# nloyfer/wgbs_tools

Hardware: AMD Instinct MI355X
Metric: CpG-sites/sec segmented (higher is better)
Workload: dtype u8 counts -> u32 prefix sums -> f32/f64 log-likelihood (bit-exact with the reference)

## Files before the change

include/wgbsseg.h:

```cpp
#ifndef WGBSSEG_H
#define WGBSSEG_H

#include <stddef.h>
#include <stdint.h>

#ifdef __cplusplus
extern "C" {
#endif

#define WGBSSEG_VERSION 270
#define WGBSSEG_MAX_CPG 65535

#define WGBSSEG_OK              0
#define WGBSSEG_E_ARG          -1
#define WGBSSEG_E_METH_GT_COV  -2
#define WGBSSEG_E_NOMEM        -3
#define WGBSSEG_E_HIP          -4
#define WGBSSEG_E_LOCI_ORDER   -5
#define WGBSSEG_E_CAPACITY     -6
#define WGBSSEG_E_STATE        -7
#define WGBSSEG_E_IO           -8

typedef struct wgbsseg_ctx wgbsseg_ctx;

typedef struct wgbsseg_params {
    float    pseudo_count;
    uint32_t max_cpg;
    uint32_t max_bp;
} wgbsseg_params;

typedef struct wgbsseg_timings {
    double scan_ms;
    double window_ms;
    double cost_ms;
    double dp_ms;
    double trace_ms;
    double total_ms;
    int64_t sites;
    int64_t pairs;
    int64_t evals;
    int64_t scan_bytes;
    int32_t max_window;
    int32_t n_stages;
    int32_t scan_launches;
    int32_t div_short;
    double  scan_main_ms;
    int64_t scan_main_bytes;
} wgbsseg_timings;

int wgbsseg_version(void);

int wgbsseg_device_count(void);

int wgbsseg_create(int device, wgbsseg_ctx** out, char* err, size_t errlen);
void wgbsseg_destroy(wgbsseg_ctx* ctx);

int wgbsseg_set_betas_host(wgbsseg_ctx* ctx, const uint8_t* const* samples, int64_t n_samples, int64_t n_sites,
                           char* err, size_t errlen);
int wgbsseg_set_lbetas_host(wgbsseg_ctx* ctx, const uint16_t* const* samples, int64_t n_samples, int64_t n_sites,
                            char* err, size_t errlen);
int wgbsseg_set_betas_device(wgbsseg_ctx* ctx, const void* base, int64_t n_samples, int64_t pitch_bytes,
                             int64_t n_sites, char* err, size_t errlen);

int wgbsseg_set_loci_host(wgbsseg_ctx* ctx, const uint32_t* loci, int64_t n_sites, char* err, size_t errlen);
int wgbsseg_set_loci_device(wgbsseg_ctx* ctx, const void* loci, int64_t n_sites, char* err, size_t errlen);

int wgbsseg_segment_chunks(wgbsseg_ctx* ctx, const int64_t* chunk_start0, const int32_t* chunk_len,
                           int64_t n_chunks, const wgbsseg_params* params,
                           int32_t* borders_out, int64_t borders_cap, int64_t* borders_off,
                           char* err, size_t errlen);

int wgbsseg_segment_regions(wgbsseg_ctx* ctx, const int64_t* region_start, const int64_t* region_end, int64_t n_regions,
                            int64_t chunk_size, const wgbsseg_params* params,
                            int32_t* borders_out, int64_t borders_cap, int64_t* borders_off, int64_t* stats,
                            char* err, size_t errlen);

typedef int (*wgbsseg_batch_fn)(void* user, const int64_t* starts, const int64_t* ends, int64_t n,
                                const int32_t** out_ptr, int64_t* out_cnt);
int wgbsseg_stitch_regions(const int64_t* region_start, const int64_t* region_end, int64_t n_regions, int64_t chunk_size,
                           wgbsseg_batch_fn fn, void* user, int32_t speculate, int32_t* borders_out, int64_t borders_cap,
                           int64_t* borders_off, int64_t* stats, char* err, size_t errlen);

int wgbsseg_first_batch_items(const int64_t* region_start, const int64_t* region_end, int64_t n_regions, int64_t chunk_size,
                              int32_t speculate, int64_t* starts, int64_t* ends, int64_t cap, int64_t* n_items, int64_t* n_chunks,
                              char* err, size_t errlen);

int wgbsseg_set_site_base(wgbsseg_ctx* ctx, int64_t site_base);

typedef struct wgbsseg_group wgbsseg_group;
int wgbsseg_plan_shares(const uint32_t* loci, int64_t n_sites, const int64_t* region_start, const int64_t* region_end,
                        int64_t n_regions, int64_t chunk_size, const wgbsseg_params* params, int32_t n_shares, int64_t halo,
                        int64_t* own_lo, int64_t* own_hi, int64_t* win_lo, int64_t* win_hi, int64_t* share_chunks,
                        int64_t* share_work, char* err, size_t errlen);
int wgbsseg_plan_shares_weighted(const uint32_t* loci, int64_t n_sites, const int64_t* region_start, const int64_t* region_end,
                                 int64_t n_regions, int64_t chunk_size, const wgbsseg_params* params, int32_t n_shares, const double* weights,
                                 int64_t halo, int64_t* own_lo, int64_t* own_hi, int64_t* win_lo, int64_t* win_hi,
                                 int64_t* share_chunks, int64_t* share_work, char* err, size_t errlen);
int wgbsseg_group_create(const int32_t* devices, int32_t n_shares, wgbsseg_group** out, char* err, size_t errlen);
void wgbsseg_group_destroy(wgbsseg_group* g);
int32_t wgbsseg_group_size(const wgbsseg_group* g);
int wgbsseg_group_plan(wgbsseg_group* g, const uint32_t* loci, int64_t n_sites, const int64_t* region_start,
                       const int64_t* region_end, int64_t n_regions, int64_t chunk_size, const wgbsseg_params* params,
                       int64_t halo, int64_t* win_lo, int64_t* win_hi, int64_t* share_chunks, int64_t* share_work,
                       char* err, size_t errlen);
int wgbsseg_group_load_host(wgbsseg_group* g, const uint8_t* const* samples, int64_t n_samples, int64_t n_sites,
                            char* err, size_t errlen);
int wgbsseg_group_load_host_async(wgbsseg_group* g, const uint8_t* const* samples, int64_t n_samples, int64_t n_sites,
                                  char* err, size_t errlen);
int wgbsseg_group_load_wait(wgbsseg_group* g, char* err, size_t errlen);
int wgbsseg_group_share_set_device(wgbsseg_group* g, int32_t share, const void* base, int64_t n_samples,
                                   int64_t pitch_bytes, char* err, size_t errlen);
int wgbsseg_group_segment_regions(wgbsseg_group* g, int32_t* borders_out, int64_t borders_cap, int64_t* borders_off,
                                  int64_t* stats, char* err, size_t errlen);

int wgbsseg_group_segment_region_range(wgbsseg_group* g, int64_t first_region, int64_t end_region, int32_t* borders_out, int64_t borders_cap,
                                       int64_t* borders_off, int64_t* stats, char* err, size_t errlen);
int wgbsseg_group_get_timings(const wgbsseg_group* g, int32_t share, wgbsseg_timings* out);

int wgbsseg_segment_chunks_host(const uint8_t* betas, int64_t n_samples, int64_t sample_pitch_bytes,
                                int64_t n_sites_total, const uint32_t* loci,
                                const int64_t* chunk_start0, const int32_t* chunk_len, int64_t n_chunks,
                                const wgbsseg_params* params, int device,
                                int32_t* borders_out, int64_t borders_cap, int64_t* borders_off,
                                char* err, size_t errlen);

int wgbsseg_prefix_sums(wgbsseg_ctx* ctx, int64_t start0, int64_t len, uint32_t* out, char* err, size_t errlen);

int wgbsseg_scan_only(wgbsseg_ctx* ctx, const int64_t* chunk_start0, const int32_t* chunk_len, int64_t n_chunks,
                      int repeat, int want_carry, double* ms_per_launch, int64_t* bytes_per_launch,
                      int64_t* carry_bytes_per_launch, char* err, size_t errlen);
// ... 106 lines not shown
```

wgbs_tools_amd/_lib.py:

```python
import ctypes as C
import os
import os.path as op

import numpy as np

HERE = op.dirname(op.abspath(__file__))
LIB_PATH = op.join(HERE, 'csrc', 'libwgbsseg.so')
if os.environ.get('WGBSSEG_LIB') and os.environ.get('WGBSSEG_ALLOW_LIB_OVERRIDE') == '1':
    LIB_PATH = os.environ['WGBSSEG_LIB']
    import sys as _sys
    print('[wgbsseg] WGBSSEG_LIB: loading %s instead of the in-tree library' % LIB_PATH, file=_sys.stderr)
SYNTH_LIB_PATH = op.join(HERE, 'csrc', 'libwgbssynth.so')

OK, E_ARG, E_METH_GT_COV, E_NOMEM, E_HIP, E_LOCI_ORDER, E_CAPACITY, E_STATE, E_IO = 0, -1, -2, -3, -4, -5, -6, -7, -8

ABI_VERSION = 270
EXPORTS = ['wgbsseg_version', 'wgbsseg_device_count', 'wgbsseg_create', 'wgbsseg_destroy',
           'wgbsseg_set_betas_host', 'wgbsseg_set_betas_device', 'wgbsseg_set_loci_host', 'wgbsseg_set_loci_device',
           'wgbsseg_segment_chunks', 'wgbsseg_segment_regions', 'wgbsseg_segment_chunks_host', 'wgbsseg_prefix_sums', 'wgbsseg_scan_only',
           'wgbsseg_get_timings', 'wgbsseg_debug_fetch', 'wgbsseg_debug_sample_terms', 'wgbsseg_debug_log2',
           'wgbsseg_debug_div', 'wgbsseg_debug_check_div', 'wgbsseg_debug_div_short', 'wgbsseg_add_loci', 'wgbsseg_add_loci_borders', 'wgbsseg_block_sums', 'wgbsseg_last_block_sums_ms',
           'wgbsseg_set_site_base', 'wgbsseg_stitch_regions', 'wgbsseg_group_create', 'wgbsseg_group_destroy', 'wgbsseg_group_size',
           'wgbsseg_group_plan', 'wgbsseg_group_load_host', 'wgbsseg_group_share_set_device', 'wgbsseg_group_segment_regions', 'wgbsseg_group_segment_region_range',
           'wgbsseg_group_get_timings', 'wgbsseg_plan_shares', 'wgbsseg_set_lbetas_host',
           'wgbsseg_convert_regions', 'wgbsseg_patbeta_create', 'wgbsseg_patbeta_feed', 'wgbsseg_patbeta_finish',
           'wgbsseg_patbeta_destroy', 'wgbsseg_patbeta_kernel_ms', 'wgbsseg_group_load_host_async', 'wgbsseg_group_load_wait',
           'wgbsseg_marker_stats', 'wgbsseg_blocks_parse', 'wgbsseg_blocks_write_table', 'wgbsseg_blocks_write_bedgraph',
           'wgbsseg_format_fixed', 'wgbsseg_bed_parse', 'wgbsseg_bed_write_annotated', 'wgbsseg_debug_canonical_float',
           'wgbsseg_first_batch_items', 'wgbsseg_plan_shares_weighted',
           'wgbsseg_homog_create', 'wgbsseg_homog_feed', 'wgbsseg_homog_finish', 'wgbsseg_homog_destroy', 'wgbsseg_homog_kernel_ms',
           'wgbsseg_debug_homog_bins',
           'wgbsseg_bimodal_create', 'wgbsseg_bimodal_feed', 'wgbsseg_bimodal_finish', 'wgbsseg_bimodal_destroy', 'wgbsseg_bimodal_kernel_ms',
           'wgbsseg_debug_bimodal_terms', 'wgbsseg_sample_stats',
           'wgbsseg_pair_ranges', 'wgbsseg_pair_hist', 'wgbsseg_pair_hist_limits',
           'wgbsseg_beta2bed', 'wgbsseg_beta2bed_pass_ms', 'wgbsseg_beta2bed_limits']


class NativeLibraryError(RuntimeError):
    pass


class SegmentorError(RuntimeError):

    def __init__(self, code, msg):
        super().__init__('[wgbsseg %d] %s' % (code, msg))
        self.code = code
        self.msg = msg


class Params(C.Structure):
    _fields_ = [('pseudo_count', C.c_float), ('max_cpg', C.c_uint32), ('max_bp', C.c_uint32)]


SAMPLE_STAT_DTYPE = np.dtype([('n_sites', np.uint64), ('meth_sum', np.uint64), ('cov_sum', np.uint64), ('covered', np.uint64),
                              ('covered_at', np.uint64), ('orphans', np.uint64), ('ratio_lo', np.uint64), ('ratio_hi', np.uint64),
                              ('max_cov', np.uint32), ('reserved', np.uint32)])

PAIR_RANGE_DTYPE = np.dtype([('n', np.uint64), ('a_min', np.float64), ('a_max', np.float64), ('b_min', np.float64), ('b_max', np.float64)])


class BedOpts(C.Structure):
    _fields_ = [('min_cov', C.c_int32), ('mean', C.c_int32), ('keep_na', C.c_int32), ('stage_bytes', C.c_int32), ('slab_sites', C.c_int64)]


class Timings(C.Structure):
    _fields_ = [('scan_ms', C.c_double), ('window_ms', C.c_double), ('cost_ms', C.c_double), ('dp_ms', C.c_double),
                ('trace_ms', C.c_double), ('total_ms', C.c_double), ('sites', C.c_int64), ('pairs', C.c_int64),
                ('evals', C.c_int64), ('scan_bytes', C.c_int64), ('max_window', C.c_int32), ('n_stages', C.c_int32),
                ('scan_launches', C.c_int32), ('div_short', C.c_int32), ('scan_main_ms', C.c_double),
                ('scan_main_bytes', C.c_int64)]

    def as_dict(self):
        return {k: getattr(self, k) for k, _ in self._fields_}


BATCH_FN = C.CFUNCTYPE(C.c_int, C.c_void_p, C.POINTER(C.c_int64), C.POINTER(C.c_int64), C.c_int64, C.POINTER(C.c_void_p),
                       C.POINTER(C.c_int64))

_lib = None
_synth = None
ERRLEN = 512
_hip_preloaded = False


def _share_hip_runtime_with_torch():
    global _hip_preloaded
    if _hip_preloaded:
        return
    _hip_preloaded = True
    import importlib.util
    import sys
    if 'torch' in sys.modules:
        return
    try:
        spec = importlib.util.find_spec('torch')
    except (ImportError, ValueError):
        spec = None
    if spec is None or not spec.origin:
        return
    cand = op.join(op.dirname(spec.origin), 'lib', 'libamdhip64.so')
    if op.isfile(cand):
        try:
            C.CDLL(cand, mode=C.RTLD_GLOBAL)
        except OSError:
            pass


def load():
    global _lib
    if _lib is not None:
        return _lib
    if not op.isfile(LIB_PATH):
        raise NativeLibraryError('%s is missing: build it with `python -m wgbs_tools_amd.build` (needs hipcc). '
                                 'There is no CPU fallback.' % LIB_PATH)
    _share_hip_runtime_with_torch()
    L = C.CDLL(LIB_PATH)
    vp, i64, i32 = C.c_void_p, C.c_int64, C.c_int
    L.wgbsseg_version.restype = i32
    got = L.wgbsseg_version()
    if got != ABI_VERSION:
        raise NativeLibraryError('%s reports ABI version %d, this binding was written against %d (include/wgbsseg.h WGBSSEG_VERSION): '
                                 'rebuild it with `python -m wgbs_tools_amd.build -f`' % (LIB_PATH, got, ABI_VERSION))
    L.wgbsseg_device_count.restype = i32
    L.wgbsseg_create.restype = i32
    L.wgbsseg_create.argtypes = [i32, C.POINTER(vp), C.c_char_p, C.c_size_t]
    L.wgbsseg_destroy.restype = None
    L.wgbsseg_destroy.argtypes = [vp]
    L.wgbsseg_set_betas_host.restype = i32
    L.wgbsseg_set_betas_host.argtypes = [vp, C.POINTER(vp), i64, i64, C.c_char_p, C.c_size_t]
    L.wgbsseg_set_lbetas_host.restype = i32
    L.wgbsseg_set_lbetas_host.argtypes = [vp, C.POINTER(vp), i64, i64, C.c_char_p, C.c_size_t]
    L.wgbsseg_set_betas_device.restype = i32
    L.wgbsseg_set_betas_device.argtypes = [vp, vp, i64, i64, i64, C.c_char_p, C.c_size_t]
    L.wgbsseg_set_loci_host.restype = i32
    L.wgbsseg_set_loci_host.argtypes = [vp, vp, i64, C.c_char_p, C.c_size_t]
    L.wgbsseg_set_loci_device.restype = i32
    L.wgbsseg_set_loci_device.argtypes = [vp, vp, i64, C.c_char_p, C.c_size_t]
    L.wgbsseg_segment_chunks.restype = i32
    L.wgbsseg_segment_chunks.argtypes = [vp, vp, vp, i64, C.POINTER(Params), vp, i64, vp, C.c_char_p, C.c_size_t]
    L.wgbsseg_segment_regions.restype = i32
    L.wgbsseg_segment_regions.argtypes = [vp, vp, vp, i64, i64, C.POINTER(Params), vp, i64, vp, vp, C.c_char_p, C.c_size_t]
    L.wgbsseg_segment_chunks_host.restype = i32
    L.wgbsseg_segment_chunks_host.argtypes = [vp, i64, i64, i64, vp, vp, vp, i64, C.POINTER(Params), i32, vp, i64, vp,
                                              C.c_char_p, C.c_size_t]
    L.wgbsseg_prefix_sums.restype = i32
    L.wgbsseg_prefix_sums.argtypes = [vp, i64, i64, vp, C.c_char_p, C.c_size_t]
    L.wgbsseg_scan_only.restype = i32
    L.wgbsseg_scan_only.argtypes = [vp, vp, vp, i64, i32, i32, C.POINTER(C.c_double), C.POINTER(i64), C.POINTER(i64), C.c_char_p, C.c_size_t]
    L.wgbsseg_get_timings.restype = i32
    L.wgbsseg_get_timings.argtypes = [vp, C.POINTER(Timings)]
    L.wgbsseg_debug_fetch.restype = i64
    L.wgbsseg_debug_fetch.argtypes = [vp, C.c_char_p, vp, i64]
    L.wgbsseg_debug_sample_terms.restype = i32
# ... 941 lines not shown
```

wgbs_tools_amd/build.py:

```python
import os
import os.path as op
import shutil
import subprocess
import sys

HERE = op.dirname(op.abspath(__file__))
CSRC = op.join(HERE, 'csrc')
ARCH = 'gfx950'
HIPFLAGS = ['--offload-arch=' + ARCH, '-O3', '-std=c++17', '-ffp-contract=off', '-fPIC', '-shared', '-pthread']

TARGETS = {
    'libwgbsseg.so': (['wgbsseg.hip'], ['owners.h', 'env.h', 'seg_kernels.h', 'block_plan.h', 'block_kernels.h', 'plain_dp.h', 'wave_prims.h', 'exact_log2.h', 'stitch.h', 'add_loci.h', 'table_io.h', 'pat_kernels.h', 'homog_kernels.h', 'bimodal_kernels.h', 'stats_kernels.h', 'pair_plan.h', 'pair_kernels.h', 'bed_fmt.h', 'bed_plan.h', 'bed_kernels.h', 'share_plan.h', '../../include/wgbsseg.h']),
    'libwgbssynth.so': (['synth.hip'], []),
}


def source_hash():
    import hashlib
    srcs, hdrs = TARGETS['libwgbsseg.so']
    h = hashlib.sha256()
    for f in sorted(op.normpath(op.join(CSRC, x)) for x in srcs + hdrs):
        with open(f, 'rb') as fh:
            h.update(fh.read())
    return h.hexdigest()[:16]


def hipcc():
    for cand in (shutil.which('hipcc'), '/opt/rocm/bin/hipcc'):
        if cand and op.isfile(cand):
            return cand
    raise RuntimeError('hipcc not found: cannot build the gfx950 libraries')


PROGRAMS = {
    'segmentor': (['segmentor_main.cpp'], ['../../include/wgbsseg.h']),
}


def _stale(out, deps):
    if not op.isfile(out):
        return True
    t = op.getmtime(out)
    return any(op.getmtime(d) > t for d in deps if op.isfile(d))


def build(force=False, verbose=False):
    built = []
    for lib, (srcs, hdrs) in TARGETS.items():
        out = op.join(CSRC, lib)
        srcp = [op.join(CSRC, s) for s in srcs]
        deps = srcp + [op.normpath(op.join(CSRC, h)) for h in hdrs]
        if not all(op.isfile(s) for s in srcp):
            continue
        if force or _stale(out, deps):
            cmd = [hipcc()] + HIPFLAGS + srcp + ['-o', out]
            if verbose:
                print(' '.join(cmd), file=sys.stderr)
            subprocess.check_call(cmd, cwd=CSRC)
            built.append(lib)
    for exe, (srcs, hdrs) in PROGRAMS.items():
        out = op.join(CSRC, exe)
        srcp = [op.join(CSRC, s) for s in srcs]
        deps = srcp + [op.normpath(op.join(CSRC, h)) for h in hdrs] + [op.join(CSRC, 'libwgbsseg.so')]
        if force or _stale(out, deps):
            cmd = [hipcc(), '-O2', '-std=c++17'] + srcp + ['-L' + CSRC, '-lwgbsseg', '-Wl,-rpath,$ORIGIN', '-o', out]
            if verbose:
                print(' '.join(cmd), file=sys.stderr)
            subprocess.check_call(cmd, cwd=CSRC)
            built.append(exe)
    return built


if __name__ == '__main__':
    print(build(force='-f' in sys.argv, verbose=True))
```

wgbs_tools_amd/csrc/seg_kernels.h:

```cpp
#pragma once
#include <hip/hip_runtime.h>
#include <stddef.h>
#include <stdint.h>
#include "exact_log2.h"
#include "wave_prims.h"

#ifndef WG_CARRY_SHIFT
#define WG_CARRY_SHIFT  7
#endif
#define WG_SCAN_STAGED  512
#define WG_CARRY_G      (1 << WG_CARRY_SHIFT)
static_assert(WG_CARRY_SHIFT >= 4 && WG_CARRY_SHIFT <= 10, "k_scan: a lane vector is 16 sites, an iteration 1024");
#define WG_BLOCK        256
#define WG_WIN_TILE     1024
#define WG_PAIR_CAP     4096
#define WG_TRACE_WIN    32768
#define WG_NARROW_WMAX  60
#define WG_MEDIUM_WMAX  252
#define WG_MEDIUM_TS    16

__device__ const wg_log_tables g_wg_tables = WG_LOG_TABLES_INIT;

__device__ __forceinline__ void wg_fast_tables_to_lds(wg_fast_tables* ft, int tid, int nthreads)
{
    const double* f = reinterpret_cast<const double*>(g_wg_tables.f_tab);
    const double* d = reinterpret_cast<const double*>(g_wg_tables.d_tab);
    double* of = reinterpret_cast<double*>(ft->f_tab);
    double* od = reinterpret_cast<double*>(ft->d_fast);
    for (int x = tid; x < 32; x += nthreads) of[x] = f[x];
    for (int x = tid; x < 128; x += nthreads) {
        double v = d[x];
        if (x == 2 * WG_FAST_CENTRE_ENTRY) v = 1.0;
        if (x == 2 * WG_FAST_CENTRE_ENTRY + 1) v = 0.0;
        od[x] = v;
    }
}

__device__ __forceinline__ void wg_lookup_tables_to_lds(wg_d2* iy, wg_d2* ky, int rows, const wg_d2* __restrict__ src, int tid, int nthreads)
{
    if (src) {
        wg_d2* dst = iy;
        for (int x = tid; x < rows * (16 + 64); x += nthreads) dst[x] = src[x];
        return;
    }
    for (int x = tid; x < rows * 16; x += nthreads) iy[x] = wg_ks_iy_entry(&g_wg_tables, rows, x);
    for (int x = tid; x < rows * 64; x += nthreads) ky[x] = wg_ks_ky_entry(&g_wg_tables, rows, x);
}

struct ChunkDesc {
    int64_t start0;
    int64_t site_off;
    int64_t carry_off;
    int64_t unit_off;
    int32_t len;
    int32_t nG;
};

struct JobView {
    const uint8_t* betas;
    int64_t pitch;
    int64_t n_total;
    const uint32_t* loci;
    const ChunkDesc* chunks;
    uint2* carry;
    uint16_t* W16;
    uint32_t* cum32;
    uint16_t* back16;
    uint16_t* umax16;
    int64_t* chunk_pairs;
    int32_t n_samples;
    int32_t n_chunks;
};

struct JobStatus {
    unsigned long long first_bad;
    unsigned long long total_pairs;
    unsigned int max_window;
    unsigned int loci_disorder;
    unsigned int overflow;
    unsigned int wide_units;
};

struct StageView {
    const int64_t* cbase;
    const uint32_t* cum0;
    const int64_t* tbaseA;
    const int64_t* tbaseB;
    int32_t stage;
    const int32_t* sb;
};

__device__ __forceinline__ uint4 wg_load16_guarded(const uint8_t* row, int64_t abs_site, int64_t n_total)
{
    if (abs_site + 8 <= n_total) return *reinterpret_cast<const uint4*>(row + 2 * abs_site);
    uint32_t w[4] = {0u, 0u, 0u, 0u};
    for (int j = 0; j < 8; j++) {
        int64_t a = abs_site + j;
        if (a < n_total) {
            uint32_t m = row[2 * a], c = row[2 * a + 1];
            w[j >> 1] |= (m | (c << 8)) << (16 * (j & 1));
        }
    }
    return make_uint4(w[0], w[1], w[2], w[3]);
}

__device__ __forceinline__ void wg_sum8(const uint4 v, uint32_t& tm, uint32_t& tt, bool& anybad)
{
    const uint32_t w[4] = {v.x, v.y, v.z, v.w};
    uint32_t sm = 0, sc = 0, ok = 0x01000100u;
#pragma unroll
    for (int d = 0; d < 4; d++) {
        const uint32_t m = w[d] & 0x00ff00ffu, c = (w[d] >> 8) & 0x00ff00ffu;
        sm += m; sc += c;
        ok &= (c | 0x01000100u) - m;
    }
    tm = (sm & 0xffffu) + (sm >> 16);
    tt = (sc & 0xffffu) + (sc >> 16);
    anybad = (ok & 0x01000100u) != 0x01000100u;
}

__device__ __noinline__ uint4 wg_blank_outside(uint4 v, int rel0, int len)
{
    uint32_t w[4] = {v.x, v.y, v.z, v.w};
#pragma unroll
    for (int j = 0; j < 8; j++) {
        const int rel = rel0 + j;
        if (rel < 0 || rel >= len) w[j >> 1] &= ~(0xffffu << (16 * (j & 1)));
    }
    return make_uint4(w[0], w[1], w[2], w[3]);
}

__device__ __noinline__ int wg_first_bad_site(uint4 v0, uint4 v1)
{
    const uint32_t w[8] = {v0.x, v0.y, v0.z, v0.w, v1.x, v1.y, v1.z, v1.w};
    int bad = 16;
    for (int j = 15; j >= 0; j--) {
        const uint32_t h = w[j >> 1] >> (16 * (j & 1));
        if ((h & 0xffu) > ((h >> 8) & 0xffu)) bad = j;
    }
    return bad;
}

__global__ __launch_bounds__(WG_BLOCK) void k_scan(JobView J, JobStatus* st)
{
    const int lane = threadIdx.x & 63;
    const int64_t rowid = (int64_t)blockIdx.x * (WG_BLOCK / 64) + (threadIdx.x >> 6);
    const int64_t nrows = (int64_t)J.n_chunks * J.n_samples;
    if (rowid >= nrows) return;
    const int c = (int)(rowid / J.n_samples);
    const int s = (int)(rowid - (int64_t)c * J.n_samples);
    const ChunkDesc cd = J.chunks[c];
    const int64_t a_abs = cd.start0 & ~15LL;
    const int head = (int)(cd.start0 - a_abs);
    const int len = cd.len;
    const int span = head + len;
    const uint4* rv = reinterpret_cast<const uint4*>(J.betas + (int64_t)s * J.pitch) + (a_abs >> 3);
    const int64_t vl = ((J.n_total - 1) >> 3) - (a_abs >> 3);
    const int vlast = vl > 0x7ffffff0 ? 0x7ffffff0 : (int)vl;
    uint2* carry = J.carry + cd.carry_off + (int64_t)s * cd.nG;
    const int A6 = (int)(a_abs & (WG_CARRY_G - 1));
    uint32_t run_m = 0, run_t = 0;
    int bad_rel = 0x7fffffff;
    if (lane == 0) carry[0] = make_uint2(0u, 0u);
    const int nit = (span + 1023) >> 10;
    __shared__ uint2 cstage[WG_BLOCK / 64][WG_SCAN_STAGED];
    uint2* cs = cstage[threadIdx.x >> 6];
    const bool staged = cd.nG <= WG_SCAN_STAGED;

    int vi = 2 * lane;
    uint4 c0 = rv[vi < vlast ? vi : vlast], c1 = rv[vi + 1 < vlast ? vi + 1 : vlast];
    for (int base = 0; base < (nit << 10); base += 1024) {
        const int vn = vi + 128;
        const uint4 m0 = rv[vn < vlast ? vn : vlast], m1 = rv[vn + 1 < vlast ? vn + 1 : vlast];
// ... 202 lines not shown
        const int64_t at = cd.site_off + k0;
        const int nv = cd.len - k0 < WG_WIN_TILE ? cd.len - k0 : WG_WIN_TILE;
        tile_info[t] = make_int4((int)(uint32_t)at, (int)(at >> 32), nv, c);
    }
}

__global__ __launch_bounds__(WG_BLOCK) void k_window_scan(JobView J, JobStatus* st, const int64_t* __restrict__ wtile_off,
                                                          const uint32_t* __restrict__ tile_tot, uint32_t* __restrict__ tile_base)
{
    __shared__ uint64_t ws[WG_BLOCK / 64];
    const int tid = threadIdx.x, lane = tid & 63, wv = tid >> 6;
    const int c = blockIdx.x;
    const int64_t t0 = wtile_off[c], t1 = wtile_off[c + 1];
    uint64_t run = 0;
    for (int64_t base = t0; base < t1; base += WG_BLOCK) {
        const int64_t t = base + tid;
        const uint64_t v = t < t1 ? (uint64_t)tile_tot[t] : 0;
        const uint64_t incl = wg_wave_incl_scan_u64(v, lane);
        if (lane == 63) ws[wv] = incl;
        __syncthreads();
        uint64_t o = 0, tot = 0;
#pragma unroll
        for (int q = 0; q < WG_BLOCK / 64; q++) { if (q < wv) o += ws[q]; tot += ws[q]; }
        __syncthreads();
        if (t < t1) tile_base[t] = (uint32_t)(run + o + incl - v);
        run += tot;
    }
    if (tid == 0) {
        J.chunk_pairs[c] = (int64_t)run;
        atomicAdd(&st->total_pairs, (unsigned long long)run);
        if (run >> 32) atomicMax(&st->overflow, 1u);
    }
}

#define WG_CUM_TILES 4
__global__ __launch_bounds__(WG_BLOCK) void k_window_cum(const uint16_t* __restrict__ W16, uint32_t* __restrict__ cum32, const int4* __restrict__ tile_info,
                                                         const uint32_t* __restrict__ tile_base, int64_t n_tiles)
{
    __shared__ uint32_t ws[WG_CUM_TILES][WG_BLOCK / 64];
    const int tid = threadIdx.x, lane = tid & 63, wv = tid >> 6;
    const int64_t t0 = (int64_t)blockIdx.x * WG_CUM_TILES;
    int4 info[WG_CUM_TILES];
    uint32_t base[WG_CUM_TILES];
#pragma unroll
    for (int q = 0; q < WG_CUM_TILES; q++) {
        const int64_t t = t0 + q < n_tiles ? t0 + q : n_tiles - 1;
        info[q] = tile_info[t];
        base[q] = tile_base[t];
        if (t0 + q >= n_tiles) info[q].z = 0;
    }
    uint2 v[WG_CUM_TILES];
#pragma unroll
    for (int q = 0; q < WG_CUM_TILES; q++) {
        const int64_t at = (int64_t)(((uint64_t)(uint32_t)info[q].y << 32) | (uint32_t)info[q].x) + 4 * tid;
        v[q] = make_uint2(0u, 0u);
        if (4 * tid < info[q].z) v[q] = *reinterpret_cast<const uint2*>(W16 + at);
    }
    uint32_t w[WG_CUM_TILES][4], tot[WG_CUM_TILES], incl[WG_CUM_TILES];
#pragma unroll
    for (int q = 0; q < WG_CUM_TILES; q++) {
        const int k = 4 * tid, n = info[q].z;
        w[q][0] = k < n ? v[q].x & 0xffffu : 0u; w[q][1] = k + 1 < n ? v[q].x >> 16 : 0u;
        w[q][2] = k + 2 < n ? v[q].y & 0xffffu : 0u; w[q][3] = k + 3 < n ? v[q].y >> 16 : 0u;
        tot[q] = w[q][0] + w[q][1] + w[q][2] + w[q][3];
        incl[q] = wg_wave_incl_scan_dpp_u32(tot[q]);
        if (lane == 63) ws[q][wv] = incl[q];
    }
    __syncthreads();
#pragma unroll
    for (int q = 0; q < WG_CUM_TILES; q++) {
        const int k = 4 * tid, n = info[q].z;
        if (k >= n) continue;
        uint32_t e = base[q] + (incl[q] - tot[q]);
#pragma unroll
        for (int x = 0; x < WG_BLOCK / 64; x++) if (x < wv) e += ws[q][x];
        const int64_t at = (int64_t)(((uint64_t)(uint32_t)info[q].y << 32) | (uint32_t)info[q].x) + k;
        uint32_t* C = cum32 + at;
        const uint4 o = make_uint4(e, e + w[q][0], e + w[q][0] + w[q][1], e + w[q][0] + w[q][1] + w[q][2]);
        if (k + 4 <= n) *reinterpret_cast<uint4*>(C) = o;
        else { C[0] = o.x; if (k + 1 < n) C[1] = o.y; if (k + 2 < n) C[2] = o.z; }
    }
}

struct PlanArgs { const int32_t* sb; int32_t TI, WA, TK, n_stages, WM; };

struct TileDesc { int32_t chunk, ka, nk, et_lo; };

__device__ __forceinline__ void wg_group_tiles(const JobView& J, const ChunkDesc& cd, const PlanArgs& P, int ka, int s1,
                                               uint32_t& nA, uint32_t& nB, uint32_t& nM)
{
    const int kb = (ka + P.TI < s1) ? ka + P.TI : s1;
    uint32_t m = 0, tb = 0, tm = 0;
    for (int k0 = ka; k0 < kb; k0 += 16) {
        const uint32_t um = J.umax16[cd.unit_off + (k0 >> 4)];
        const int nk = (kb - k0 < 16) ? kb - k0 : 16;
        m = um > m ? um : m;
        if (um <= (uint32_t)P.WM) tm += 1u;
        else tb += ((uint32_t)(nk - 1) + um + (uint32_t)P.TK - 1u) / (uint32_t)P.TK;
    }
    const bool narrow = m <= (uint32_t)P.WA;
    nA = narrow ? 1u : 0u;
    nB = narrow ? 0u : tb;
    nM = narrow ? 0u : tm;
}

__global__ __launch_bounds__(WG_BLOCK) void k_tile_count(JobView J, PlanArgs P, uint32_t* __restrict__ cntA, uint32_t* __restrict__ cntB,
                                                         uint32_t* __restrict__ cntM)
{
    __shared__ uint32_t wa[WG_BLOCK / 64], wb[WG_BLOCK / 64], wm[WG_BLOCK / 64];
    const int tid = threadIdx.x, lane = tid & 63, wv = tid >> 6;
    const int c = blockIdx.x, stg = blockIdx.y;
    const ChunkDesc cd = J.chunks[c];
    const int s0 = P.sb[stg];
    uint32_t a = 0, b = 0, m = 0;
    if (s0 < cd.len) {
        const int s1 = (P.sb[stg + 1] < cd.len) ? P.sb[stg + 1] : cd.len;
        const int nU = (s1 - s0 + P.TI - 1) / P.TI;
        for (int u = tid; u < nU; u += WG_BLOCK) {
            uint32_t na, nb, nm;
            wg_group_tiles(J, cd, P, s0 + u * P.TI, s1, na, nb, nm);
            a += na; b += nb; m += nm;
        }
    }
    for (int o = 32; o > 0; o >>= 1) { a += (uint32_t)__shfl_down((int)a, o); b += (uint32_t)__shfl_down((int)b, o); m += (uint32_t)__shfl_down((int)m, o); }
    if (lane == 0) { wa[wv] = a; wb[wv] = b; wm[wv] = m; }
    __syncthreads();
    if (tid == 0) {
        uint32_t ta = 0, tb = 0, tm = 0;
        for (int q = 0; q < WG_BLOCK / 64; q++) { ta += wa[q]; tb += wb[q]; tm += wm[q]; }
        cntA[(int64_t)stg * J.n_chunks + c] = ta;
        cntB[(int64_t)stg * J.n_chunks + c] = tb;
        cntM[(int64_t)stg * J.n_chunks + c] = tm;
    }
}

#define WG_PLAN_BLOCK 256
__global__ __launch_bounds__(WG_PLAN_BLOCK) void k_stage_plan(JobView J, PlanArgs P, const uint32_t* __restrict__ cntA,
                                                         const uint32_t* __restrict__ cntB, const uint32_t* __restrict__ cntM, int64_t* cbase, uint32_t* cum0,
                                                         int64_t* tbaseA, int64_t* tbaseB, int64_t* tbaseM, int64_t* stage_pairs, int64_t* stage_tiles)
{
    __shared__ uint64_t wa[WG_PLAN_BLOCK / 64], wb[WG_PLAN_BLOCK / 64], wc[WG_PLAN_BLOCK / 64], wd[WG_PLAN_BLOCK / 64];
    const int tid = threadIdx.x, lane = tid & 63, wv = tid >> 6;
    const int stg = blockIdx.x;
    const int nC = J.n_chunks;
    uint64_t runA = 0, runB = 0, runC = 0, runD = 0;
    for (int base = 0; base < nC; base += WG_PLAN_BLOCK) {
        const int c = base + tid;
        uint64_t sz = 0, nt = 0, nu = 0, nm = 0;
        uint32_t c0 = 0;
        if (c < nC) {
            const ChunkDesc cd = J.chunks[c];
            const int64_t s0 = P.sb[stg];
            if (s0 < cd.len) {
                const int64_t s1 = (P.sb[stg + 1] < cd.len) ? P.sb[stg + 1] : cd.len;
                c0 = J.cum32[cd.site_off + s0];
                const uint64_t cend = (s1 < cd.len) ? (uint64_t)J.cum32[cd.site_off + s1] : (uint64_t)J.chunk_pairs[c];
                sz = cend - c0;
                nt = cntA ? (uint64_t)cntA[(int64_t)stg * nC + c] : (uint64_t)((s1 - s0 + P.TI - 1) / P.TI);
                nu = cntA ? (uint64_t)cntB[(int64_t)stg * nC + c] : 0;
                nm = cntA ? (uint64_t)cntM[(int64_t)stg * nC + c] : 0;
            }
        }
        const uint64_t ia = wg_wave_incl_scan_u64(sz, lane), ib = wg_wave_incl_scan_u64(nt, lane), ic = wg_wave_incl_scan_u64(nu, lane),
                       id = wg_wave_incl_scan_u64(nm, lane);
        if (lane == 63) { wa[wv] = ia; wb[wv] = ib; wc[wv] = ic; wd[wv] = id; }
        __syncthreads();
        uint64_t oa = 0, ob = 0, oc = 0, od = 0, ta = 0, tb2 = 0, tc = 0, td = 0;
#pragma unroll
        for (int q = 0; q < WG_PLAN_BLOCK / 64; q++) {
            if (q < wv) { oa += wa[q]; ob += wb[q]; oc += wc[q]; od += wd[q]; }
            ta += wa[q]; tb2 += wb[q]; tc += wc[q]; td += wd[q];
        }
        __syncthreads();
        if (c < nC) {
            cbase[(int64_t)stg * nC + c] = (int64_t)(runA + oa + ia - sz);
            cum0[(int64_t)stg * nC + c] = c0;
            tbaseA[(int64_t)stg * (nC + 1) + c] = (int64_t)(runB + ob + ib - nt);
            tbaseB[(int64_t)stg * (nC + 1) + c] = (int64_t)(runC + oc + ic - nu);
            tbaseM[(int64_t)stg * (nC + 1) + c] = (int64_t)(runD + od + id - nm);
        }
        runA += ta; runB += tb2; runC += tc; runD += td;
    }
    if (tid == 0) {
        tbaseA[(int64_t)stg * (nC + 1) + nC] = (int64_t)runB;
        tbaseB[(int64_t)stg * (nC + 1) + nC] = (int64_t)runC;
        tbaseM[(int64_t)stg * (nC + 1) + nC] = (int64_t)runD;
        stage_pairs[stg] = (int64_t)runA;
        stage_tiles[3 * stg] = (int64_t)runB;
        stage_tiles[3 * stg + 1] = (int64_t)runC;
        stage_tiles[3 * stg + 2] = (int64_t)runD;
    }
}

__global__ __launch_bounds__(WG_BLOCK) void k_tile_emit(JobView J, PlanArgs P, int stg, const int64_t* __restrict__ tbaseA,
                                                        const int64_t* __restrict__ tbaseB, const int64_t* __restrict__ tbaseM,
                                                        TileDesc* __restrict__ tilesA, TileDesc* __restrict__ tilesB, TileDesc* __restrict__ tilesM)
{
    __shared__ uint32_t wa[WG_BLOCK / 64], wb[WG_BLOCK / 64], wm[WG_BLOCK / 64];
    const int tid = threadIdx.x, lane = tid & 63, wv = tid >> 6;
    const int c = blockIdx.x;
    const int nC = J.n_chunks;
    const ChunkDesc cd = J.chunks[c];
    const int s0 = P.sb[stg];
    if (s0 >= cd.len) return;
    const int s1 = (P.sb[stg + 1] < cd.len) ? P.sb[stg + 1] : cd.len;
    const int nU = (s1 - s0 + P.TI - 1) / P.TI;
    int64_t runA = tbaseA[(int64_t)stg * (nC + 1) + c], runB = tbaseB[(int64_t)stg * (nC + 1) + c], runM = tbaseM[(int64_t)stg * (nC + 1) + c];
    for (int base = 0; base < nU; base += WG_BLOCK) {
        const int u = base + tid;
        const int ka = s0 + u * P.TI;
        uint32_t na = 0, nb = 0, nm = 0;
        if (u < nU) wg_group_tiles(J, cd, P, ka, s1, na, nb, nm);
        const uint32_t ia = wg_wave_incl_scan_dpp_u32(na), ib = wg_wave_incl_scan_dpp_u32(nb), im = wg_wave_incl_scan_dpp_u32(nm);
        if (lane == 63) { wa[wv] = ia; wb[wv] = ib; wm[wv] = im; }
        __syncthreads();
        uint32_t oa = 0, ob = 0, om = 0, ta = 0, tb = 0, tm = 0;
#pragma unroll
        for (int q = 0; q < WG_BLOCK / 64; q++) { if (q < wv) { oa += wa[q]; ob += wb[q]; om += wm[q]; } ta += wa[q]; tb += wb[q]; tm += wm[q]; }
        __syncthreads();
        if (u < nU) {
            const int kb = (ka + P.TI < s1) ? ka + P.TI : s1;
            if (na) {
                TileDesc d = {c, ka, kb - ka, 0};
                tilesA[runA + oa + ia - na] = d;
            } else {
                int64_t o = runB + ob + ib - nb, om2 = runM + om + im - nm;
                for (int k0 = ka; k0 < kb; k0 += 16) {
                    const uint32_t um = J.umax16[cd.unit_off + (k0 >> 4)];
                    const int nk = (kb - k0 < 16) ? kb - k0 : 16;
                    if (um <= (uint32_t)P.WM) { TileDesc d = {c, k0, nk, 0}; tilesM[om2++] = d; continue; }
                    const int kt = (int)(((uint32_t)(nk - 1) + um + (uint32_t)P.TK - 1u) / (uint32_t)P.TK);
                    for (int e = 0; e < kt; e++) { TileDesc d = {c, k0, nk, k0 + e * P.TK}; tilesB[o++] = d; }
                }
            }
        }
        runA += ta; runB += tb; runM += tm;
    }
}

struct CostArgs {
    float pc, pc2;
    int32_t NS;
    int32_t rows;
    const wg_d2* tab;
    int32_t xcd_group;
    int32_t cmap;
    uint32_t* finished;
};

__global__ __launch_bounds__(64) void k_stage_gate(const uint32_t* __restrict__ finished, uint32_t need, long long max_ticks)
{
    if (threadIdx.x != 0) return;
    const long long t0 = wall_clock64();
    while (__hip_atomic_load(finished, __ATOMIC_RELAXED, __HIP_MEMORY_SCOPE_AGENT) < need && wall_clock64() - t0 < max_ticks) __builtin_amdgcn_s_sleep(8);
}

__device__ __forceinline__ void wg_stage_prefix_row(uint2* __restrict__ dst, const uint8_t* __restrict__ row,
                                                    const uint2* __restrict__ carry, const ChunkDesc& cd,
                                                    int64_t n_total, int A, int x0, int cnt0, int lane)
{
    const int cnt = x0 + cnt0;
    const int64_t abs0 = cd.start0 + A;
    const uint2 c0 = carry[(abs0 >> WG_CARRY_SHIFT) - (cd.start0 >> WG_CARRY_SHIFT)];
    uint32_t run_m = c0.x, run_t = c0.y;
    const int64_t al = abs0 & ~3LL;
    const int hs = (int)(abs0 - al);
    for (int p0 = 0; p0 < cnt + hs; p0 += 256) {
        const int sidx = p0 + lane * 4;
        const int64_t a = al + sidx;
        uint32_t w0 = 0, w1 = 0;
        if (sidx < cnt + hs) {
            if (a + 4 <= n_total) {
                const uint2 v = *reinterpret_cast<const uint2*>(row + 2 * a);
                w0 = v.x; w1 = v.y;
            } else {
                for (int j = 0; j < 4; j++) if (a + j < n_total) {
                    const uint32_t h = (uint32_t)row[2 * (a + j)] | ((uint32_t)row[2 * (a + j) + 1] << 8);
                    if (j < 2) w0 |= h << (16 * j); else w1 |= h << (16 * (j - 2));
                }
            }
        }
        uint32_t m[4], t[4];
        uint32_t tot = 0;
#pragma unroll
        for (int j = 0; j < 4; j++) {
            const uint32_t h = ((j < 2) ? w0 : w1) >> (16 * (j & 1));
            const int x = sidx + j - hs;
            const bool in = x >= 0 && (A + x) < cd.len;
// ... 626 lines not shown
    "v_cmp_gt_f64 vcc, v[6:7], v[2:3]\n"                \
    "v_max_f64 v[2:3], v[2:3], v[6:7]\n"                \
    "v_cndmask_b32_e32 v4, v4, v45, vcc\n"              \
    "v_readlane_b32 s20, v2, %[" P "]\n"                \
    "v_readlane_b32 s21, v3, %[" P "]\n"                \
    "v_add_u32_e32 v45, 1, v45\n"
#define WG_DP32W_MOVE  "v_cndmask_b32_e64 v2, v2, v42, s[24:25]\n" "v_cndmask_b32_e64 v3, v3, v43, s[24:25]\n" "v_cndmask_b32_e64 v4, v4, v44, s[24:25]\n"
#define WG_DP32W_REARM "v_cndmask_b32_e64 v42, v42, 0, s[24:25]\n" "v_cndmask_b32_e64 v43, v43, v40, s[24:25]\n"
#define WG_DP32W_CAPT  "v_cndmask_b32_e64 v5, v5, v4, s[24:25]\n"
#define WG_DP32W_BLOCK(R0, R1, R2, R3, R4, R5, R6, R7)                                                     \
            WG_DP32W_CORE(R0, "p0") WG_DP32W_MOVE                                                          \
            WG_DP32W_CORE(R1, "p1") WG_DP32W_REARM                                                         \
            WG_DP32W_CORE(R2, "p2") WG_DP64L_MASK("ml0", "mh0")                                            \
            WG_DP32W_CORE(R3, "p3") WG_DP32W_CAPT                                                          \
            WG_DP32W_CORE(R4, "p4") WG_DP32W_MOVE                                                          \
            WG_DP32W_CORE(R5, "p5") WG_DP32W_REARM                                                         \
            WG_DP32W_CORE(R6, "p6") WG_DP64L_MASK("ml1", "mh1")                                            \
            WG_DP32W_CORE(R7, "p7") WG_DP32W_CAPT
#define WG_DP32W_OPERANDS(V0, V1, V2, V3, V4, V5, V6, V7)                                                  \
            : "+{v[2:3]}"(best), "+{v4}"(arg), "+{v5}"(tbk), "+{s[20:21]}"(Mk), "+{s[24:25]}"(mask), "+{v45}"(kk), "+{v[42:43]}"(bestB), "+{v44}"(argB) \
            : V0(cur[0]), V1(cur[1]), V2(cur[2]), V3(cur[3]), V4(cur[4]), V5(cur[5]), V6(cur[6]), V7(cur[7]), "{v40}"(ninf_splat), \
              [p0] "n"(G + 0), [p1] "n"(G + 1), [p2] "n"(G + 2), [p3] "n"(G + 3), [p4] "n"(G + 4), [p5] "n"(G + 5), [p6] "n"(G + 6), [p7] "n"(G + 7), \
              [ml0] "n"((int)(uint32_t)(0xfull << G)), [mh0] "n"((int)(uint32_t)((0xfull << G) >> 32)),   \
              [ml1] "n"((int)(uint32_t)(0xfull << (G + 4))), [mh1] "n"((int)(uint32_t)((0xfull << (G + 4)) >> 32)) \
            : "v6", "v7", "vcc"

template <int G, int SET>
__device__ __forceinline__ void wg_dp_group32w(double& best, int32_t& arg, double& bestB, int32_t& argB, uint32_t& tbk, double& Mk, uint64_t& mask,
                                               uint32_t& kk, const double (&cur)[8], const uint32_t ninf_splat)
{
    if (SET == 0) asm volatile(WG_DP32W_BLOCK("v[8:9]", "v[10:11]", "v[12:13]", "v[14:15]", "v[16:17]", "v[18:19]", "v[20:21]", "v[22:23]")
                               WG_DP32W_OPERANDS("{v[8:9]}", "{v[10:11]}", "{v[12:13]}", "{v[14:15]}", "{v[16:17]}", "{v[18:19]}", "{v[20:21]}", "{v[22:23]}"));
    else          asm volatile(WG_DP32W_BLOCK("v[24:25]", "v[26:27]", "v[28:29]", "v[30:31]", "v[32:33]", "v[34:35]", "v[36:37]", "v[38:39]")
                               WG_DP32W_OPERANDS("{v[24:25]}", "{v[26:27]}", "{v[28:29]}", "{v[30:31]}", "{v[32:33]}", "{v[34:35]}", "{v[36:37]}", "{v[38:39]}"));
}

template <int STP0>
__device__ __forceinline__ void wg_dp_batch32w(double& best, int32_t& arg, double& bestB, int32_t& argB, uint32_t& tbk, double& Mk,
                                               const double* __restrict__ my, const int base, const int lane)
{
    const uint32_t ninf_hi = 0xfff00000u;
    const double NEG_INF = -__builtin_inf();
    double Ms = wg_readlane_f64(Mk, 0);
    uint32_t kk = (uint32_t)base;
    uint64_t mask = 0;
    double ra[8], rb[8];
#pragma unroll
    for (int u = 0; u < 8; u++) ra[u] = my[u * 64];
#pragma unroll
    for (int u = 0; u < 8; u++) rb[u] = my[(8 + u) * 64];
    wg_dp_group32w<STP0 + 0, 0>(best, arg, bestB, argB, tbk, Ms, mask, kk, ra, ninf_hi);
#pragma unroll
    for (int u = 0; u < 8; u++) ra[u] = my[(16 + u) * 64];
    wg_dp_group32w<STP0 + 8, 1>(best, arg, bestB, argB, tbk, Ms, mask, kk, rb, ninf_hi);
#pragma unroll
    for (int u = 0; u < 8; u++) rb[u] = my[(24 + u) * 64];
    wg_dp_group32w<STP0 + 16, 0>(best, arg, bestB, argB, tbk, Ms, mask, kk, ra, ninf_hi);
    wg_dp_group32w<STP0 + 24, 1>(best, arg, bestB, argB, tbk, Ms, mask, kk, rb, ninf_hi);
    const bool last4 = lane >= STP0 + 28 && lane < STP0 + 32;
    best = last4 ? bestB : best;
    arg = last4 ? argB : arg;
    bestB = last4 ? NEG_INF : bestB;
    Mk = Ms;
}

template <int NW, int BL, bool LEAN = false>
__global__ __launch_bounds__(64 * (1 + NW)) void k_dp(JobView J, StageView SV, const double* __restrict__ cost, DpArgs A,
                                                      double* __restrict__ state, int64_t state_stride)
{
    constexpr bool WIDEJOB = BL < 64;
    constexpr int SLOT = BL * 64 * (WIDEJOB ? 2 : 1);
    extern __shared__ __attribute__((aligned(16))) char smem_dp[];
    double* slots = reinterpret_cast<double*>(smem_dp);
    double* Mring = slots + 2 * SLOT;
    double* pendLB = Mring + 128;
    int32_t* pendLA = reinterpret_cast<int32_t*>(pendLB + 64);
    uint32_t* kinds = reinterpret_cast<uint32_t*>(pendLA + 64);
    uint32_t* metaC = kinds + 4;
    uint16_t* metaW = reinterpret_cast<uint16_t*>(metaC + WG_DP_META_RING);
    const int lane = threadIdx.x & 63;
    const int wvl = (int)(threadIdx.x >> 6);
    const bool worker = wvl != 0;
    const int lw = wvl - 1;
    const int c = blockIdx.x;
    const int nC = J.n_chunks;
    const ChunkDesc cd = J.chunks[c];
    const int s0 = SV.sb[SV.stage];
    if (s0 >= cd.len) return;
    const int s1 = (SV.sb[SV.stage + 1] < cd.len) ? SV.sb[SV.stage + 1] : cd.len;
    const int rmask = A.ringN - 1;
    double* gs = state + (int64_t)c * state_stride;
    double* pendB = gs + WG_DP_STATE_HDR;
    int32_t* pendA = reinterpret_cast<int32_t*>(pendB + A.ringN);
    const double* cb = cost + SV.cbase[(int64_t)SV.stage * nC + c];
    const uint32_t cum0 = SV.cum0[(int64_t)SV.stage * nC + c];
    const uint16_t* Wp = J.W16 + cd.site_off;
    const uint32_t* Cp = J.cum32 + cd.site_off;
    const double NEG_INF = -__builtin_inf();
    const int nb = (s1 - s0 + BL - 1) / BL;

    if (!worker) __builtin_amdgcn_s_setprio(3);
    double best = NEG_INF, bestB = NEG_INF;
    int32_t arg = 0, argB = 0;
    double Mk = 0.0;
    DpRows<NW, BL> rows;
    DpRefill<NW> refill;
    uint32_t fm_prev = 0, fm_cur = 0, fm_n1 = 0;
    constexpr int RB = WG_DP_META_REGION / BL;
    if (worker) {
        if (WIDEJOB && s0 == 0)
            for (int x = lw * 64 + lane; x < A.ringN; x += 64 * NW) pendB[x] = NEG_INF;
        wg_dp_refill_issue<NW>(refill, Wp, Cp, cum0, s0, s1, lane, lw);
        wg_dp_refill_commit<NW>(refill, metaW, metaC, 0, lane, lw);
        wg_dp_refill_issue<NW>(refill, Wp, Cp, cum0, s0 + WG_DP_META_REGION, s1, lane, lw);
        wg_dp_refill_commit<NW>(refill, metaW, metaC, WG_DP_META_REGION, lane, lw);
        if (WIDEJOB && lw == 0 && lane < BL) {
            double v = NEG_INF;
            int32_t a = 0;
            if (s0 != 0) {
                const int sl = (s0 + lane) & rmask;
                v = wg_ld_l2_f64(pendB + sl); a = wg_ld_l2_i32(pendA + sl);
                pendB[sl] = NEG_INF;
            }
            pendLB[lane] = v; pendLA[lane] = a;
        }
    } else if (s0 != 0) {
        Mk = gs[0];
        best = gs[1 + lane];
        arg = (int32_t)__double_as_longlong(gs[65 + lane]);
        if (WIDEJOB) {
            bestB = gs[129 + lane];
            argB = (int32_t)__double_as_longlong(gs[193 + lane]);
        }
        asm volatile("" : "+v"(Mk), "+v"(best), "+v"(arg), "+v"(bestB), "+v"(argB));
    }
    __syncthreads();
    if (worker) {
        wg_dp_rows_issue<NW, BL>(rows, cb, wg_dp_meta_lds<BL>(metaW, metaC, 0, lane), s0, lane, lw);
        wg_dp_rows_commit<NW, BL>(rows, slots, slots + BL * 64, kinds, lane, lw);
        fm_cur = rows.fmax;
        if (nb > 1) { wg_dp_rows_issue<NW, BL>(rows, cb, wg_dp_meta_lds<BL>(metaW, metaC, BL, lane), s0 + BL, lane, lw); fm_n1 = rows.fmax; }
    }
    __syncthreads();

#define WG_DP_BARRIER asm volatile("s_waitcnt lgkmcnt(0)\n\ts_barrier" ::: "memory")
    WG_DP_T(uint64_t dbg_wait = 0; uint64_t dbg_vm = 0; uint64_t dbg_commit = 0; uint64_t dbg_issue = 0; const uint64_t dbg_t0 = __builtin_amdgcn_s_memtime();)
    WG_DP_T(const int dbg_mode = A.pad[1];
            if (worker && (dbg_mode & 1)) return;)
    if (worker) {
      for (int b = 0; b < nb; b++) {
        const int base = s0 + b * BL;
        {
            const bool fetch = WIDEJOB && b + 1 < nb && lw == 0 && lane < BL;
            const int fsl = (base + BL + lane) & rmask;
            double fv = NEG_INF;
            int32_t fa = 0;
            if (fetch) {
                fv = wg_ld_l2_f64(pendB + fsl); fa = wg_ld_l2_i32(pendA + fsl);
                pendB[fsl] = NEG_INF;
            }
            if (b >= RB && b % RB == 0)      wg_dp_refill_issue<NW>(refill, Wp, Cp, cum0, s0 + (b / RB + 1) * WG_DP_META_REGION, s1, lane, lw);
            else if (b > RB && b % RB == 1)  wg_dp_refill_commit<NW>(refill, metaW, metaC, (b / RB + 1) * WG_DP_META_REGION, lane, lw);
            if (WIDEJOB && b >= 1 && fm_prev > 128u)
                wg_dp_far<NW, BL>(cb, Wp, Cp, cum0, base - BL, s1, Mring, pendB, pendA, rmask, lane, lw);
            WG_DP_T(const uint64_t tc0 = __builtin_amdgcn_s_memtime(); asm volatile("s_waitcnt vmcnt(0)" ::: "memory"); dbg_vm += __builtin_amdgcn_s_memtime() - tc0;)
            if (b + 1 < nb WG_DP_T(&& !(dbg_mode & 2)))
                wg_dp_rows_commit<NW, BL>(rows, slots + (size_t)((b + 1) & 1) * SLOT, slots + (size_t)((b + 1) & 1) * SLOT + BL * 64,
                                          kinds + ((b + 1) & 1), lane, lw);
            WG_DP_T(asm volatile("s_waitcnt lgkmcnt(0)" ::: "memory"); dbg_commit += __builtin_amdgcn_s_memtime() - tc0;)
            if (fetch) {
                pendLB[((b + 1) & 1) * 32 + lane] = fv;
                pendLA[((b + 1) & 1) * 32 + lane] = fa;
// ... 70 lines not shown
                else           wg_dp_wide_batch32<32>(best, arg, bestB, argB, tbk, Mfin, Mk, my, myB, base, lane);
                tbk = (uint32_t)(base + d + 1) - tbk;
                if (fin) Mring[(base + d + 1) & 127] = Mfin;
            }
            if (fin && base + d < s1) J.back16[cd.site_off + base + d] = (uint16_t)tbk;
        }
        WG_DP_T(const uint64_t tb0 = __builtin_amdgcn_s_memtime();)
        WG_DP_BARRIER;
        WG_DP_T(dbg_wait += __builtin_amdgcn_s_memtime() - tb0;)
      }
    }
#undef WG_DP_BARRIER
    WG_DP_T(if (s1 >= cd.len && lane == 0 && wvl <= 1) {
        gs[2 * wvl] = (double)(__builtin_amdgcn_s_memtime() - dbg_t0);
        gs[2 * wvl + 1] = (double)dbg_wait;
        if (wvl == 1) { gs[4] = (double)dbg_vm; gs[5] = (double)dbg_commit; gs[6] = (double)dbg_issue; }
    })
    WG_DP_T(if (s1 >= cd.len && lane == 0) {
        gs[8 + wvl] = (double)__builtin_amdgcn_s_getreg((31 << 11) | 4);
        if (wvl == 0) { gs[16] = (double)__builtin_amdgcn_s_getreg((31 << 11) | 20); gs[17] = (double)dbg_t0; gs[18] = (double)__builtin_amdgcn_s_memtime(); }
        gs[20 + wvl] = (double)dbg_wait;
        gs[40 + wvl] = (double)dbg_issue;
    })
    if (WIDEJOB && worker && fm_prev > 128u)
        wg_dp_far<NW, BL>(cb, Wp, Cp, cum0, s0 + (nb - 1) * BL, s1, Mring, pendB, pendA, rmask, lane, lw);
    if (!worker && s1 < cd.len) {
        if (lane == 0) gs[0] = Mk;
        gs[1 + lane] = best;
        gs[65 + lane] = __longlong_as_double((long long)arg);
        if (WIDEJOB) {
            gs[129 + lane] = bestB;
            gs[193 + lane] = __longlong_as_double((long long)argB);
        }
    }
}

template <int NW>
struct Dp16Rows { static constexpr int PER = (16 + NW - 1) / NW; double va[PER]; };

template <int NW>
__device__ __forceinline__ void wg_dp16_issue(Dp16Rows<NW>& R, const double* __restrict__ cb, const uint16_t* __restrict__ metaW,
                                              const uint32_t* __restrict__ metaC, int base_rel, int base, int lane, int lw)
{
    const int x = (base_rel + lane) & (WG_DP_META_RING - 1);
    const uint32_t w = lane < 16 ? (uint32_t)metaW[x] : 0u;
    const uint32_t rel = metaC[x];
    const int stp0 = base & 63;
#pragma unroll
    for (int q = 0; q < Dp16Rows<NW>::PER; q++) {
        const int sidx = lw + q * NW;
        R.va[q] = -__builtin_inf();
        if (sidx < 16) {
            const uint32_t f = (uint32_t)__builtin_amdgcn_readlane((int)w, sidx);
            const uint32_t r = (uint32_t)__builtin_amdgcn_readlane((int)rel, sidx);
            const uint32_t j = (uint32_t)(lane - stp0 - sidx) & 63u;
            if (j < f) R.va[q] = cb[(int64_t)r + j];
        }
    }
}

template <int NW>
__device__ __forceinline__ void wg_dp16_commit(const Dp16Rows<NW>& R, double* __restrict__ slot, int lane, int lw)
{
#pragma unroll
    for (int q = 0; q < Dp16Rows<NW>::PER; q++) {
        const int sidx = lw + q * NW;
        if (sidx < 16) slot[sidx * 64 + lane] = R.va[q];
    }
}

template <int NW>
__global__ __launch_bounds__(64 * (1 + NW)) void k_dp16(JobView J, StageView SV, const double* __restrict__ cost,
                                                         double* __restrict__ state, int64_t state_stride)
{
    constexpr int BL = 16, D = 4;
    constexpr int RB = WG_DP_META_REGION / BL;
    extern __shared__ __attribute__((aligned(16))) char smem_dp[];
    double* slots = reinterpret_cast<double*>(smem_dp);
    uint32_t* metaC = reinterpret_cast<uint32_t*>(slots + 2 * BL * 64);
    uint16_t* metaW = reinterpret_cast<uint16_t*>(metaC + WG_DP_META_RING);
    const int lane = threadIdx.x & 63;
    const bool worker = threadIdx.x >= 64;
    const int lw = (int)(threadIdx.x >> 6) - 1;
    const int c = blockIdx.x;
    const int nC = J.n_chunks;
    const ChunkDesc cd = J.chunks[c];
    const int s0 = SV.sb[SV.stage];
    if (s0 >= cd.len) return;
    const int s1 = (SV.sb[SV.stage + 1] < cd.len) ? SV.sb[SV.stage + 1] : cd.len;
    double* gs = state + (int64_t)c * state_stride;
    const double* cb = cost + SV.cbase[(int64_t)SV.stage * nC + c];
    const uint32_t cum0 = SV.cum0[(int64_t)SV.stage * nC + c];
    const uint16_t* Wp = J.W16 + cd.site_off;
    const uint32_t* Cp = J.cum32 + cd.site_off;
    const int nb = (s1 - s0 + BL - 1) / BL;

    if (!worker) __builtin_amdgcn_s_setprio(3);
    double best = -__builtin_inf();
    int32_t arg = 0;
    double Mk = 0.0;
    Dp16Rows<NW> r0, r1, r2, r3;
    DpRefill<NW> refill;
    if (worker) {
        wg_dp_refill_issue<NW>(refill, Wp, Cp, cum0, s0, s1, lane, lw);
        wg_dp_refill_commit<NW>(refill, metaW, metaC, 0, lane, lw);
        wg_dp_refill_issue<NW>(refill, Wp, Cp, cum0, s0 + WG_DP_META_REGION, s1, lane, lw);
        wg_dp_refill_commit<NW>(refill, metaW, metaC, WG_DP_META_REGION, lane, lw);
    } else if (s0 != 0) {
        Mk = gs[0];
        best = gs[1 + lane];
        arg = (int32_t)__double_as_longlong(gs[65 + lane]);
        asm volatile("" : "+v"(Mk), "+v"(best), "+v"(arg));
    }
    __syncthreads();
    if (worker) {
        wg_dp16_issue<NW>(r0, cb, metaW, metaC, 0, s0, lane, lw);
        wg_dp16_commit<NW>(r0, slots, lane, lw);
        if (1 < nb) wg_dp16_issue<NW>(r1, cb, metaW, metaC, 1 * BL, s0 + 1 * BL, lane, lw);
        if (2 < nb) wg_dp16_issue<NW>(r2, cb, metaW, metaC, 2 * BL, s0 + 2 * BL, lane, lw);
        if (3 < nb) wg_dp16_issue<NW>(r3, cb, metaW, metaC, 3 * BL, s0 + 3 * BL, lane, lw);
        if (4 < nb) wg_dp16_issue<NW>(r0, cb, metaW, metaC, 4 * BL, s0 + 4 * BL, lane, lw);
    }
    __syncthreads();

    const uint32_t ninf_hi = 0xfff00000u;
    uint32_t tbk = 0;
#define WG_DP16_WORKER(Q, RNEXT)                                                                                           \
    if (b4 + (Q) < nb) {                                                                                                   \
        const int b = b4 + (Q);                                                                                            \
        if (b >= RB && b % RB == 0)      wg_dp_refill_issue<NW>(refill, Wp, Cp, cum0, s0 + (b / RB + 1) * WG_DP_META_REGION, s1, lane, lw); \
        else if (b > RB && b % RB == 1)  wg_dp_refill_commit<NW>(refill, metaW, metaC, (b / RB + 1) * WG_DP_META_REGION, lane, lw); \
        if (b + 1 < nb) wg_dp16_commit<NW>(RNEXT, slots + (size_t)((b + 1) & 1) * (BL * 64), lane, lw);                       \
        if (b + 1 + D < nb) wg_dp16_issue<NW>(RNEXT, cb, metaW, metaC, (b + 1 + D) * BL, s0 + (b + 1 + D) * BL, lane, lw);     \
        asm volatile("s_waitcnt lgkmcnt(0)\n\ts_barrier" ::: "memory");                                                    \
    }
#define WG_DP16_REC(Q)                                                                                                     \
    if (b4 + (Q) < nb) {                                                                                                   \
        const int b = b4 + (Q);                                                                                            \
        const double* my = slots + (size_t)(b & 1) * (BL * 64) + lane;                                                     \
        double ra[8], rb[8];                                                                                               \
        _Pragma("unroll") for (int u = 0; u < 8; u++) { ra[u] = my[u * 64]; rb[u] = my[(8 + u) * 64]; }                    \
        double Ms = wg_readlane_f64(Mk, 0);          \
        wg_dp_group64<16 * (Q), 0>(best, arg, tbk, Ms, ra, ninf_hi);                                                       \
        wg_dp_group64<16 * (Q) + 8, 1>(best, arg, tbk, Ms, rb, ninf_hi);                                                   \
        Mk = Ms;                                                                                                           \
        asm volatile("s_waitcnt lgkmcnt(0)\n\ts_barrier" ::: "memory");                                                    \
    }
    if (worker) {
        for (int b4 = 0; b4 < nb; b4 += 4) { WG_DP16_WORKER(0, r1) WG_DP16_WORKER(1, r2) WG_DP16_WORKER(2, r3) WG_DP16_WORKER(3, r0) }
    } else {
        for (int b4 = 0; b4 < nb; b4 += 4) {
            WG_DP16_REC(0) WG_DP16_REC(1) WG_DP16_REC(2) WG_DP16_REC(3)
            const int i = s0 + b4 * BL + lane;
            const uint32_t len = (((uint32_t)lane - tbk) & 63u) + 1u;
            if (i < s1) J.back16[cd.site_off + i] = (uint16_t)len;
            tbk = 0;
        }
    }
#undef WG_DP16_WORKER
#undef WG_DP16_REC
    if (!worker && s1 < cd.len) {
        if (lane == 0) gs[0] = Mk;
        gs[1 + lane] = best;
        gs[65 + lane] = __longlong_as_double((long long)arg);
    }
}

__device__ __forceinline__ int wg_trace_step(const uint16_t* win, int i, int wlo)
{
    int stepb = (int)win[i - 1 - wlo];
    if (stepb < 1 || stepb > i) stepb = i;
    return i - stepb;
// ... 267 lines not shown
```

wgbs_tools_amd/csrc/wgbsseg.hip:

```cpp
#include <hip/hip_runtime.h>
#include <algorithm>
#include <atomic>
#include <cerrno>
#include <chrono>
#include <cstdarg>
#include <cstdio>
#include <cstdlib>
#include <cstring>
#include <deque>
#include <functional>
#include <initializer_list>
#include <memory>
#include <string>
#include <thread>
#include <vector>
#include <pthread.h>
#include <sched.h>
#include <sys/mman.h>
#include <unistd.h>
#if defined(__x86_64__) && !defined(__HIP_DEVICE_COMPILE__)
#include <emmintrin.h>
#endif

#include "../../include/wgbsseg.h"
// ... 3 lines not shown
#include "share_plan.h"
#include "block_kernels.h"
#include "pat_kernels.h"
#include "homog_kernels.h"
#include "bimodal_kernels.h"
#include "stats_kernels.h"
#include "pair_kernels.h"
#include "bed_kernels.h"
#include "plain_dp.h"
#include "stitch.h"
#include "add_loci.h"
#include "table_io.h"

namespace {

void set_err(char* err, size_t errlen, const char* fmt, ...)
{
    if (!err || !errlen) return;
    va_list ap;
    va_start(ap, fmt);
    vsnprintf(err, errlen, fmt, ap);
    va_end(ap);
}

#define HIP_TRY(expr)                                                                              \
    do {                                                                                           \
        hipError_t e__ = (expr);                                                                   \
        if (e__ != hipSuccess) {                                                                   \
            set_err(err, errlen, "HIP error %d (%s) at %s:%d: %s", (int)e__, hipGetErrorString(e__), \
                    __FILE__, __LINE__, #expr);                                                    \
            return WGBSSEG_E_HIP;                                                                  \
        }                                                                                          \
    } while (0)

hipError_t set_kernel_attributes();
inline int ceil_pow2(int v) { int r = 1; while (r < v) r <<= 1; return r; }
inline int64_t round_up(int64_t v, int64_t m) { return (v + m - 1) / m * m; }

}

#define WG_MAX_CPUS 8192
struct NearCpus { std::vector<unsigned long> bits; bool valid = false; };

enum BatchEvent { EV_BEGIN, EV_WINDOWS, EV_SCAN_END, EV_PLAN, EV_TRACE0, EV_TRACE1, EV_HOME, EV_STATS, EV_VALIDATE0, EV_VALIDATE1, EV_SCAN0, EV_SCAN1, EV_UPLOADED, EV_COUNT };

struct wgbsseg_ctx {
    int device = 0;
    NearCpus near_cpus;
    Stream sA, sB, sC;
    Stream sA2;
    DevBuf betas_own, loci_own;
    const uint8_t* betas = nullptr;
    int64_t pitch = 0, n_total = 0;
    int32_t elem = 1;
    int64_t site_base = 0;
    int32_t n_samples = 0;
    const uint32_t* loci = nullptr;
    int64_t n_loci = 0;
    DevBuf chunks, wtile, carry, W16, cum32, back16, chunk_pairs, status, tile_tot, tile_base, tile_chunk;
    DevBuf plan_cbase, plan_cum0, plan_tbase, plan_pairs, plan_tiles, plan_cnt, umax16;
    std::vector<PinnedBuf> pinned;
    std::vector<PinnedBuf> up_stage;
    DevBuf tiles[3], cost[3], stage_ctr, dpstate, tmp_borders, nb, boff, out_borders[2], edges, lookup;
    DevBuf dbg_a, dbg_b, dbg_c;
    int out_par = 0;
    Event evS;
    Event evD;
    bool out_pending = false;
    bool batch_open = false;
    std::vector<wg_d2> h_lookup;
    float lookup_pc = -1.0f;
    int lookup_rows[3] = {-1, -1, -1};
    Event ev[EV_COUNT];
    PinnedBuf h_status;
    PinnedBuf h_job, h_pieces, h_sb;
    PinnedBuf h_out;
    std::vector<Event> ev_cost0, ev_cost1, ev_dp0, ev_dp1, ev_fork, ev_join;
    wgbsseg_timings tim = {};
    int64_t last_sites = 0, last_pairs = 0;
    int32_t last_stages = 0;
    bool last_valid = false;
    long long cost_budget_bytes = 0;
    int force_stages = 0;
    bool counted_live = false;
    double stage_gate_wide_evals = 100000.0, stage_min_evals_per_step = 21000.0;
    bool stage_gate_shared = false;
    int stage_gate = 768, last_stage_pct = -1, force_dp_mode = 0, force_ns = 0, force_ti = 0;
    double last_block_sums_ms = 0.0;
    int64_t table_blocks = 0;
    bool accumulate = false;
    std::vector<std::pair<int64_t, int64_t>> validated;
    DevBuf scan_pieces, divcheck, plan_sb;
    DevBuf bs_plan, bs_desc, bs_out;
    DevBuf mk_out, cv_in, cv_out;
    DevBuf st_ranges, st_parts;
    DevBuf ph_pairs, ph_edges, ph_out;
    DevBuf bed_tab, bed_mult, bed_wg, bed_out[2];
    PinnedBuf bed_home[2], bed_tot;
    Event bed_ev[2][4];
    double bed_len_ms = 0.0, bed_emit_ms = 0.0;
    std::vector<int32_t> h_stage_bounds;
    float divs_pc = -1.0f;
    bool divs_ok = false;
    int64_t last_dp_chunks = 0, last_dp_stride = 0;
    float divs_m_pc = -1.0f;
    bool divs_m_ok = false;
    bool divs_enabled = true, bs_general = false;
    int64_t scan_piece_sites = 4096;
    int medium_wmax = WG_MEDIUM_WMAX;
    bool dp_wlean = true, early = true, speculate = true, batch_marks = false;
    ~wgbsseg_ctx() { (void)hipSetDevice(device); (void)hipDeviceSynchronize(); }
};

namespace {

bool device_local_cpus(int device, NearCpus* out)
{
    out->valid = false;
    if (!env_flag("WGBSSEG_UPLOAD_PIN", true)) return false;
    char bus[64] = {0};
    if (hipDeviceGetPCIBusId(bus, (int)sizeof bus, device) != hipSuccess) { (void)hipGetLastError(); return false; }
    for (char* q = bus; *q; q++) if (*q >= 'A' && *q <= 'F') *q = (char)(*q - 'A' + 'a');
    char path[160];
    snprintf(path, sizeof path, "/sys/bus/pci/devices/%s/local_cpulist", bus);
    FILE* f = fopen(path, "r");
    if (!f) return false;
    char line[8192] = {0};
    const bool got = fgets(line, (int)sizeof line, f) != nullptr;
    fclose(f);
    if (!got) return false;
    const size_t bytes = CPU_ALLOC_SIZE(WG_MAX_CPUS);
    std::vector<unsigned long> allowed(bytes / sizeof(unsigned long), 0ul);
    out->bits.assign(bytes / sizeof(unsigned long), 0ul);
    cpu_set_t* A = reinterpret_cast<cpu_set_t*>(allowed.data());
    cpu_set_t* L = reinterpret_cast<cpu_set_t*>(out->bits.data());
    if (sched_getaffinity(0, bytes, A) != 0) return false;
    int n_local = 0;
    for (const char* q = line; *q;) {
        while (*q == ',' || *q == ' ' || *q == '\n') q++;
        if (*q < '0' || *q > '9') break;
        char* end = nullptr;
        long a = strtol(q, &end, 10), b = a;
        if (*end == '-') b = strtol(end + 1, &end, 10);
        for (long x = a; x <= b && x < WG_MAX_CPUS; x++) if (CPU_ISSET_S((int)x, bytes, A)) { CPU_SET_S((int)x, bytes, L); n_local++; }
        q = end;
    }
    if (n_local == 0 || n_local == CPU_COUNT_S(bytes, A)) return false;
    out->valid = true;
    return true;
}
inline void pin_to(const NearCpus& n)
{
    if (n.valid) (void)pthread_setaffinity_np(pthread_self(), n.bits.size() * sizeof(unsigned long), reinterpret_cast<const cpu_set_t*>(n.bits.data()));
}
struct FillMode { bool populate = true, nt = true; };
inline void fill_piece(void* dst, const uint8_t* src, size_t n, const FillMode& m)
{
#ifdef MADV_POPULATE_READ
    if (m.populate) {
        const uintptr_t a = reinterpret_cast<uintptr_t>(src) & ~(uintptr_t)4095, b = (reinterpret_cast<uintptr_t>(src) + n + 4095) & ~(uintptr_t)4095;
        (void)madvise(reinterpret_cast<void*>(a), b - a, MADV_POPULATE_READ);
    }
#endif
#if defined(__x86_64__) && !defined(__HIP_DEVICE_COMPILE__)
    if (m.nt && (reinterpret_cast<uintptr_t>(dst) & 15) == 0) {
        __m128i* d = reinterpret_cast<__m128i*>(dst);
        const __m128i* s = reinterpret_cast<const __m128i*>(src);
        size_t v = n >> 6;
        for (; v > 0; v--, s += 4, d += 4) {
            const __m128i x0 = _mm_loadu_si128(s), x1 = _mm_loadu_si128(s + 1), x2 = _mm_loadu_si128(s + 2), x3 = _mm_loadu_si128(s + 3);
            _mm_stream_si128(d, x0); _mm_stream_si128(d + 1, x1); _mm_stream_si128(d + 2, x2); _mm_stream_si128(d + 3, x3);
        }
        _mm_sfence();
        const size_t done = n & ~(size_t)63;
        if (n > done) memcpy(static_cast<char*>(dst) + done, src + done, n - done);
        return;
    }
#endif
    memcpy(dst, src, n);
}
struct UploadPlan {
    int64_t piece = 0, ppr = 0, n_tasks = 0;
    int T = 1, depth = 2;
    bool piece_major = false;
// ... 96 lines not shown
    std::atomic<int64_t> pieces_done(0);
    std::mutex mu;
    auto complete = [&](int64_t task) {
        const int64_t p = task / n_rows;
        if (rows_done[(size_t)p].fetch_add(1) + 1 == (int)n_rows) {
            std::lock_guard<std::mutex> lk(mu);
            int64_t d = pieces_done.load();
            while (d < u.ppr && rows_done[(size_t)d].load() == (int)n_rows) d++;
            pieces_done.store(d);
            ready_sites.store(std::min<int64_t>(d * u.piece, row_bytes) / 2);
        }
    };
    const std::vector<hipError_t> terr = run_upload(c, u, dst, dst_pitch, rows, n_rows, row_bytes, complete);
    for (int t = 0; t < u.T; t++)
        if (terr[(size_t)t] != hipSuccess) { msg = std::string("HIP error during the upload: ") + hipGetErrorString(terr[(size_t)t]); return WGBSSEG_E_HIP; }
    ready_sites.store(row_bytes / 2);
    if (profiling()) fprintf(stderr, "[wgbsseg] betas to the device (streaming): %.1f ms, %.1f GB/s (%d upload threads x %d pieces of %lld KB%s%s%s)\n", (wall_s() - t0) * 1e3,
                             (double)row_bytes * n_rows / (wall_s() - t0) * 1e-9, u.T, u.depth, (long long)(u.piece >> 10), c->near_cpus.valid ? ", on the device's CPUs" : "",
                             u.fill.populate ? ", pages mapped per piece" : "", u.fill.nt ? ", non-temporal fill" : "");
    return WGBSSEG_OK;
}

}

extern "C" {

int wgbsseg_version(void) { return WGBSSEG_VERSION; }

int wgbsseg_device_count(void)
{
    int n = 0;
    if (hipGetDeviceCount(&n) != hipSuccess) return 0;
    return n;
}

}
namespace {
std::atomic<int> g_live_ctx[64];

int check_device(int device, char* err, size_t errlen)
{
    int n = 0;
    hipError_t e = hipGetDeviceCount(&n);
    if (e != hipSuccess || n <= 0) {
        set_err(err, errlen, "no HIP device available (%s); libwgbsseg has no CPU fallback", hipGetErrorString(e));
        return WGBSSEG_E_HIP;
    }
    if (device < 0 || device >= n) { set_err(err, errlen, "device %d out of range (0..%d)", device, n - 1); return WGBSSEG_E_ARG; }
    HIP_TRY(hipSetDevice(device));
    hipDeviceProp_t prop;
    HIP_TRY(hipGetDeviceProperties(&prop, device));
    if (!strstr(prop.gcnArchName, "gfx950")) {
        set_err(err, errlen, "device %d is %s; this library carries gfx950 code only", device, prop.gcnArchName);
        return WGBSSEG_E_HIP;
    }
    return WGBSSEG_OK;
}

int create_ctx(int device, bool scan_low_priority, wgbsseg_ctx** out, char* err, size_t errlen)
{
    if (!out) { set_err(err, errlen, "out is NULL"); return WGBSSEG_E_ARG; }
    *out = nullptr;
    const int rc = check_device(device, err, errlen);
    if (rc != WGBSSEG_OK) return rc;
    HIP_TRY(set_kernel_attributes());
    std::unique_ptr<wgbsseg_ctx> c(new (std::nothrow) wgbsseg_ctx());
    if (!c) { set_err(err, errlen, "out of host memory"); return WGBSSEG_E_NOMEM; }
    c->device = device;
    (void)device_local_cpus(device, &c->near_cpus);
    HIP_TRY(c->sA.create());
    {
        int lo_p = 0, hi_p = 0;
        (void)hipDeviceGetStreamPriorityRange(&lo_p, &hi_p);
        HIP_TRY(c->sB.create(hi_p));
        HIP_TRY(scan_low_priority ? c->sC.create(lo_p) : c->sC.create());
    }
    HIP_TRY(c->sA2.create());
    HIP_TRY(c->evD.create(false));
    HIP_TRY(c->evS.create(false));
    for (auto& v : c->ev) HIP_TRY(v.create());
    const long long budget_mb = env_int("WGBSSEG_COST_BUDGET_MB", 0);
    c->cost_budget_bytes = (budget_mb > 0 ? budget_mb : 6144LL) << 20;
    c->force_stages = (int)env_int("WGBSSEG_FORCE_STAGES", 0);
    c->stage_gate = (int)env_int("WGBSSEG_STAGE_GATE", c->stage_gate, 0);
    c->stage_gate_shared = env_flag("WGBSSEG_STAGE_GATE_SHARED", false);
    c->stage_gate_wide_evals = env_double("WGBSSEG_STAGE_GATE_WIDE_EVALS", c->stage_gate_wide_evals);
    c->stage_min_evals_per_step = env_double("WGBSSEG_STAGE_MIN_EVALS", c->stage_min_evals_per_step);
    if (env_int("WGBSSEG_LAST_STAGE_PCT", -1) != -1) c->last_stage_pct = (int)env_int("WGBSSEG_LAST_STAGE_PCT", -1, 5, 800);
    c->force_dp_mode = (int)env_int("WGBSSEG_DP_MODE", 0, 0, 2);
    c->force_ns = (int)env_int("WGBSSEG_NS", 0);
    c->force_ti = (int)env_int("WGBSSEG_TI", 0);
    c->bs_general = env_flag("WGBSSEG_BLOCK_SUMS_GENERAL", false);
    c->divs_enabled = env_flag("WGBSSEG_DIV_SHORT", true);
    { const long long sp = env_int("WGBSSEG_SCAN_PIECE_SITES", 0); if (sp >= 1024) c->scan_piece_sites = sp & ~1023LL; }
    const int wm = (int)env_int("WGBSSEG_MEDIUM_WMAX", WG_MEDIUM_WMAX, 0, WG_MEDIUM_WMAX);
    c->medium_wmax = wm > WG_NARROW_WMAX ? wm : 0;
    c->dp_wlean = env_flag("WGBSSEG_DP_WLEAN", true);
    c->early = !env_flag("WGBSSEG_NO_EARLY", false);
    c->speculate = !env_flag("WGBSSEG_NO_SPECULATION", false);
    c->batch_marks = env_int("WGBSSEG_PROFILE", 0) >= 2;
    g_live_ctx[device & 63].fetch_add(1, std::memory_order_relaxed);
    c->counted_live = true;
    *out = c.release();
    return WGBSSEG_OK;
}
}
extern "C" {

int wgbsseg_create(int device, wgbsseg_ctx** out, char* err, size_t errlen) { return create_ctx(device, true, out, err, errlen); }

void wgbsseg_destroy(wgbsseg_ctx* c)
{
    if (!c) return;
    if (c->counted_live) g_live_ctx[c->device & 63].fetch_sub(1, std::memory_order_relaxed);
    const double t0 = wall_s();
    delete c;
    if (profiling()) fprintf(stderr, "[wgbsseg] destroy: %.1f ms\n", (wall_s() - t0) * 1e3);
}

static hipError_t own_rows(wgbsseg_ctx* c, int64_t n_samples, int64_t n_sites, int elem)
{
    const int64_t pitch = round_up(2 * elem * n_sites, 256) + 256;
    const hipError_t e = c->betas_own.ensure((size_t)pitch * (size_t)n_samples);
    if (e != hipSuccess) return e;
    c->betas = c->betas_own.as<uint8_t>();
    c->pitch = pitch; c->n_total = n_sites; c->n_samples = (int32_t)n_samples; c->elem = elem;
    c->last_valid = false;
    return hipSuccess;
}

static int set_rows_host(wgbsseg_ctx* c, const uint8_t* const* samples, int64_t n_samples, int64_t n_sites, int elem, char* err, size_t errlen)
{
    if (!c || !samples || n_samples < 1 || n_sites < 1) { set_err(err, errlen, "bad arguments to set_betas_host"); return WGBSSEG_E_ARG; }
    for (int64_t s = 0; s < n_samples; s++)
        if (!samples[s]) { set_err(err, errlen, "samples[%lld] is NULL", (long long)s); return WGBSSEG_E_ARG; }
    HIP_TRY(hipSetDevice(c->device));
    HIP_TRY(own_rows(c, n_samples, n_sites, elem));
    return upload_rows(c, c->betas_own.as<uint8_t>(), c->pitch, samples, n_samples, 2 * elem * n_sites, "betas", err, errlen);
}

int wgbsseg_set_betas_host(wgbsseg_ctx* c, const uint8_t* const* samples, int64_t n_samples, int64_t n_sites,
                           char* err, size_t errlen)
{
    return set_rows_host(c, samples, n_samples, n_sites, 1, err, errlen);
}

int wgbsseg_set_lbetas_host(wgbsseg_ctx* c, const uint16_t* const* samples, int64_t n_samples, int64_t n_sites,
                            char* err, size_t errlen)
{
    return set_rows_host(c, reinterpret_cast<const uint8_t* const*>(samples), n_samples, n_sites, 2, err, errlen);
}

int wgbsseg_set_betas_device(wgbsseg_ctx* c, const void* base, int64_t n_samples, int64_t pitch_bytes, int64_t n_sites,
                             char* err, size_t errlen)
{
    if (!c || !base || n_samples < 1 || n_sites < 1 || pitch_bytes < 2 * n_sites) { set_err(err, errlen, "bad arguments to set_betas_device"); return WGBSSEG_E_ARG; }
    if (((uintptr_t)base & 15) || (pitch_bytes & 15)) { set_err(err, errlen, "device betas base and pitch must be multiples of 16 bytes"); return WGBSSEG_E_ARG; }
    c->betas = reinterpret_cast<const uint8_t*>(base);
    c->pitch = pitch_bytes; c->n_total = n_sites; c->n_samples = (int32_t)n_samples; c->elem = 1;
    c->last_valid = false;
    return WGBSSEG_OK;
}

int wgbsseg_set_loci_host(wgbsseg_ctx* c, const uint32_t* loci, int64_t n_sites, char* err, size_t errlen)
{
    if (!c || !loci || n_sites < 1) { set_err(err, errlen, "bad arguments to set_loci_host"); return WGBSSEG_E_ARG; }
// ... 240 lines not shown
}

void grow_events(std::vector<Event>& v, size_t n)
{
    while (v.size() < n) { v.emplace_back(); (void)v.back().create(); }
}

typedef std::function<int32_t*(int64_t)> BorderAlloc;

struct EarlyOut {
    int64_t n_lead = 0;
    bool dest_device_visible = false;
    const int32_t* edges = nullptr;
    bool pending = false;
};
int wait_pending_output(wgbsseg_ctx* c, char* err, size_t errlen)
{
    if (!c->out_pending) return WGBSSEG_OK;
    c->out_pending = false;
    HIP_TRY(hipSetDevice(c->device));
    HIP_TRY(hipEventSynchronize(c->evD));
    return WGBSSEG_OK;
}

int plain_segment_chunk(wgbsseg_ctx* c, int64_t start0, int32_t n, const wgbsseg_params* P, std::vector<int32_t>& borders, char* err, size_t errlen)
{
    const int32_t W = (int32_t)std::min<int64_t>(P->max_cpg, n);
    int64_t budget_rows = std::max<int64_t>((int64_t)W + 255, (1LL << 30) / ((int64_t)W * 8));
    const long long cap_rows = env_int("WGBSSEG_PLAIN_RING_ROWS", 0);
    if (cap_rows > 0) budget_rows = std::max<int64_t>((int64_t)W, (int64_t)cap_rows);
    const int32_t R = (int32_t)std::min<int64_t>(n, budget_rows);
    const int32_t band = R >= n ? n : R - (W - 1);
    DevBuf buf, M, T, bad;
    if (buf.ensure((size_t)W * (size_t)R * 8) != hipSuccess || M.ensure((size_t)(n + 1) * 8) != hipSuccess || T.ensure((size_t)(n + 1) * 4) != hipSuccess ||
        bad.ensure(8) != hipSuccess) {
        (void)hipGetLastError();
        set_err(err, errlen, "out of device memory for the plain recurrence of a chunk with non-ascending loci (%d sites, max_cpg %d)", (int)n, (int)W);
        return WGBSSEG_E_NOMEM;
    }
    JobStatus st = {};
    st.first_bad = ~0ULL;
    HIP_TRY(hipMemcpyAsync(bad.p, &st.first_bad, 8, hipMemcpyHostToDevice, c->sA));
    PlainArgs A = {c->betas, c->pitch, c->n_total, c->n_samples, c->loci, start0, n, W, P->max_bp, P->pseudo_count, P->pseudo_count + P->pseudo_count,
                   R, buf.as<double>(), M.as<double>(), T.as<int32_t>(), bad.as<unsigned long long>()};
    for (int32_t b0 = 0; b0 < n; b0 += band) {
        const int32_t b1 = (int32_t)std::min<int64_t>(n, (int64_t)b0 + band);
        hipLaunchKernelGGL(k_plain_rows, dim3((unsigned)((b1 - b0 + WG_BLOCK - 1) / WG_BLOCK)), dim3(WG_BLOCK), 0, c->sA, A, b0, b1);
        HIP_TRY(hipGetLastError());
        hipLaunchKernelGGL(k_plain_dp, dim3(1), dim3(WG_BLOCK), 0, c->sA, A, b0, b1);
        HIP_TRY(hipGetLastError());
    }
    std::vector<int32_t> hT((size_t)n + 1);
    HIP_TRY(hipMemcpyAsync(hT.data(), T.p, (size_t)(n + 1) * 4, hipMemcpyDeviceToHost, c->sA));
    HIP_TRY(hipMemcpyAsync(&st.first_bad, bad.p, 8, hipMemcpyDeviceToHost, c->sA));
    HIP_TRY(hipStreamSynchronize(c->sA));
    if (st.first_bad != ~0ULL) return report_bad_site(c, st, err, errlen);
    borders.clear();
    int32_t i = n;
    borders.push_back(i);
    while (i > 0) {
        const int32_t t = hT[(size_t)i];
        const int32_t nx = t > 0 ? t : 0;
        if (nx >= i) { set_err(err, errlen, "internal: back-pointer %d at step %d of a plain recurrence", (int)t, (int)i); return WGBSSEG_E_STATE; }
        i = nx;
        borders.push_back(i);
    }
    std::reverse(borders.begin(), borders.end());
    return WGBSSEG_OK;
}


struct BatchPlan {
    int Wmax = 0;
    int WA = 0;
    int WMED = 0;
    int term_mode[3] = {};
    int rows[3] = {};
    int TI = 64;
    int NS[3] = {1, 1, 1};
    size_t lds[3] = {};
    int n_stages = 1;
    bool gated = false;
    int last_pct = 100;
    const int32_t* sb = nullptr;
    bool all_narrow = false;
    std::vector<int64_t> stage_pairs, stage_tiles;
    int dp_mode = 0;
    int ringN = 0; int64_t state_stride = 0;
    int nbuf = 1;
};

size_t cost_lds(const BatchPlan& p, int ti, int cls, int ns)
{
    const int wm = cls == 2 ? WG_MEDIUM_WMAX : WG_NARROW_WMAX;
    const size_t rows = cls == 1 ? ((((size_t)ns * (WG_WIDE_TK + 1 + WG_WIDE_TS + 1) + 1) & ~(size_t)1) * 8)
                                 : ((((size_t)ns * (ti + wm + 1) + 3) & ~(size_t)3) * 4);
    const size_t tabs = p.term_mode[cls] == 2 ? (size_t)p.rows[cls] * (16 + 64) * sizeof(wg_d2) : sizeof(wg_fast_tables);
    return tabs + rows + (size_t)(ti + 1) * 16 + 32 + (cls == 1 ? 0 : ((size_t)ti * wm >> 3) + 8);
}

int plan_tiles(const wgbsseg_ctx* c, const Job& job, const JobStatus& st, float pc, BatchPlan& p, char* err, size_t errlen)
{
    p.Wmax = (int)st.max_window;
    p.WA = std::min(p.Wmax, WG_NARROW_WMAX);
    p.WMED = c->medium_wmax;
    const int tmA = wg_term_mode(pc);
    const int tmB = (tmA == 2 && 255.0 * std::max(p.Wmax, 1) >= 0x1p21) ? 1 : tmA;
    p.term_mode[0] = p.term_mode[2] = tmA;
    p.term_mode[1] = tmB;
    p.rows[0] = tmA == 2 ? wg_lookup_rows(pc, 255.0 * WG_NARROW_WMAX) : 0;
    p.rows[1] = tmB == 2 ? wg_lookup_rows(pc, 255.0 * std::max(p.Wmax, 1)) : 0;
    p.rows[2] = tmA == 2 ? wg_lookup_rows(pc, 255.0 * WG_MEDIUM_WMAX) : 0;
    if (p.rows[0] > WG_KY_KMIN + 1 || p.rows[1] > WG_KY_KMIN + 1 || p.rows[2] > WG_KY_KMIN + 1) {
        set_err(err, errlen, "internal: %d / %d / %d lookup rows", p.rows[0], p.rows[1], p.rows[2]);
        return WGBSSEG_E_ARG;
    }
    const int Nsmp = (int)c->n_samples;
    const double Favg = (double)(int64_t)st.total_pairs / (double)std::max<int64_t>(1, job.sites);
    const int ti128_max_n = 16;
    double best = -1;
    for (int ti = 128; ti >= 16; ti >>= 1) {
        if (c->force_ti > 0 && ti != c->force_ti) continue;
        for (int ns : {Nsmp, 32, 16, 8, 4}) {
            if (ns > Nsmp) continue;
            if (ti == 128 && (ns != Nsmp || (c->force_ti != 128 && Nsmp > ti128_max_n))) continue;
            if (c->force_ns > 0 && ns != std::min(c->force_ns, Nsmp)) continue;
            const size_t l = cost_lds(p, ti, 0, ns);
            if (l > 64 * 1024) continue;
            const int wgs = (int)std::min<size_t>(ti == 128 ? 8 : 5, (160 * 1024) / (size_t)round_up((int64_t)l, 1280));
            const double q = ti * std::min<double>(Favg, p.WA), eff = q / (256.0 * std::ceil(q / 256.0));
            const double groups = std::ceil((double)Nsmp / ns);
            const double score = wgs * eff / (1.0 + 0.02 * (groups - 1)) * (1.0 + 0.04 * (ti / 16));
            if (score > best) { best = score; p.TI = ti; p.NS[0] = ns; }
        }
    }
    if (best < 0) { p.TI = 16; p.NS[0] = 1; }
    auto pick_ns = [&](int cls, int ti, int max_wgs, bool forced) {
        int pick = 1;
        double top = -1;
        for (int ns : {Nsmp, 32, 16, 8, 4, 1}) {
            if (ns > Nsmp) continue;
            if (forced && c->force_ns > 0 && ns != std::min(c->force_ns, Nsmp)) continue;
            const size_t l = cost_lds(p, ti, cls, ns);
            if (l > 64 * 1024) continue;
            const int wgs = (int)std::min<size_t>(max_wgs, (160 * 1024) / (size_t)round_up((int64_t)l, 1280));
            const double score = wgs / (1.0 + 0.02 * (std::ceil((double)Nsmp / ns) - 1));
            if (score > top) { top = score; pick = ns; }
        }
        return pick;
    };
    p.NS[1] = pick_ns(1, WG_WIDE_TS, 4, true);
    p.NS[2] = pick_ns(2, WG_MEDIUM_TS, 5, false);
    const int tile_ti[3] = {p.TI, WG_WIDE_TS, WG_MEDIUM_TS};
    for (int k = 0; k < 3; k++) p.lds[k] = (size_t)round_up((int64_t)cost_lds(p, tile_ti[k], k, p.NS[k]), 16);
    return WGBSSEG_OK;
}

void plan_stages(wgbsseg_ctx* c, const Job& job, const JobStatus& st, BatchPlan& p)
{
    const int64_t total_pairs = (int64_t)st.total_pairs;
    const long long bytes = total_pairs * 8;
    int n_stages = (int)std::max<long long>(1, (bytes + c->cost_budget_bytes - 1) / c->cost_budget_bytes);
    int n_long = 0;
    for (const ChunkDesc& d : job.h) n_long += d.len >= 8192;
    const bool worth = (double)total_pairs * c->n_samples >= (double)job.max_len * c->stage_min_evals_per_step;
    if (job.max_len >= 8192) n_stages = std::max(n_stages, n_long <= 160 && worth ? 8 : 1);
    if (c->force_stages > 0) n_stages = c->force_stages;
    n_stages = std::min<int>(n_stages, std::max(1, (job.max_len + 63) / 64));
    p.all_narrow = p.Wmax <= WG_NARROW_WMAX;
    const double evals_per_step = (double)total_pairs * c->n_samples / std::max<double>(1.0, (double)job.max_len);
    p.gated = c->stage_gate > 0 && n_stages > 1 && (p.all_narrow || evals_per_step >= c->stage_gate_wide_evals || c->stage_gate_shared) &&
              (c->stage_gate_shared || g_live_ctx[c->device & 63].load(std::memory_order_relaxed) == 1);
    p.last_pct = !p.gated ? 100 : (c->last_stage_pct > 0 ? c->last_stage_pct : (evals_per_step <= 52500.0 ? 300 : 100));
    const double parts = n_stages > 1 ? (double)(n_stages - 1) + p.last_pct / 100.0 : 1.0;
    const int S = (int)round_up((int64_t)std::ceil((double)job.max_len / parts), 64);
    n_stages = std::min<int>(n_stages, (job.max_len + S - 1) / S);
    std::vector<int32_t>& sb = c->h_stage_bounds;
    sb.resize((size_t)n_stages + 1);
    for (int q = 0; q < n_stages; q++) sb[(size_t)q] = (int32_t)std::min<int64_t>((int64_t)q * S, job.max_len);
    sb[(size_t)n_stages] = (int32_t)job.max_len;
    p.sb = sb.data();
    p.n_stages = n_stages;
    p.stage_pairs.assign((size_t)n_stages, 0);
    p.stage_tiles.assign((size_t)n_stages * 3, 0);
    if (p.all_narrow) {
        for (int stg = 0; stg < n_stages; stg++) {
            int64_t nt = 0, sites_in = 0;
            for (const ChunkDesc& d : job.h) {
                const int64_t s0 = sb[(size_t)stg], s1 = std::min<int64_t>(sb[(size_t)stg + 1], d.len);
                if (s1 > s0) { nt += (s1 - s0 + p.TI - 1) / p.TI; sites_in += s1 - s0; }
            }
            p.stage_tiles[3 * (size_t)stg] = nt;
            p.stage_pairs[(size_t)stg] = n_stages == 1 ? total_pairs : std::min<int64_t>(total_pairs, sites_in * std::max(p.Wmax, 1));
        }
    }
    p.nbuf = n_stages > 1 ? (p.gated && n_stages > 2 ? 3 : 2) : 1;
    p.dp_mode = std::max(p.Wmax > 512 ? 2 : (p.Wmax > 64 ? 1 : 0), c->force_dp_mode);
    p.ringN = p.dp_mode ? ceil_pow2(p.Wmax + 128) : 0;
    p.state_stride = round_up(WG_DP_STATE_HDR + (int64_t)p.ringN + (p.ringN + 1) / 2, 2);
}

int queue_div_check(wgbsseg_ctx* c, float pc, int wmax, void* dst, char* err, size_t errlen)
{
    HIP_TRY(c->divcheck.ensure(4));
    HIP_TRY(hipMemsetAsync(c->divcheck.p, 0, 4, c->sA));
    const int max_total = 255 * wmax;
    hipLaunchKernelGGL(k_check_div, dim3((unsigned)max_total + 1), dim3(WG_BLOCK), 0, c->sA, pc, pc + pc, max_total, c->divcheck.as<unsigned int>());
    HIP_TRY(hipGetLastError());
    HIP_TRY(hipMemcpyAsync(dst, c->divcheck.p, 4, hipMemcpyDeviceToHost, c->sA));
    return WGBSSEG_OK;
}

struct Batch {
    wgbsseg_ctx* c = nullptr;
    const int64_t* chunk_start0 = nullptr; const int32_t* chunk_len = nullptr; int64_t n_chunks = 0;
    const BorderAlloc* alloc = nullptr; int64_t* borders_off = nullptr; EarlyOut* early = nullptr;
    bool allow_plain = true;
    wgbsseg_params P = {};
    Job job;
    int nC = 0; int64_t J = 0;
    JobStatus* hst = nullptr;
    JobStatus st = {};
    BatchPlan plan;
    CostArgs ca[3];
    std::vector<int64_t> tile0[3];
    DevBuf* outb = nullptr; size_t out_head = 0;
    bool marks = false;
    double hm[8] = {0, 0, 0, 0, 0, 0, 0, 0};
    void mark(int i) { if (marks) hm[i] = wall_s(); }

    int front(char* err, size_t errlen);
    int disorder_exit(char* err, size_t errlen);
    int tile_plan(char* err, size_t errlen);
    int stages(char* err, size_t errlen);
    int deliver(char* err, size_t errlen);
    int timings(char* err, size_t errlen);
};

int segment_chunks_impl(wgbsseg_ctx* c, const int64_t* chunk_start0, const int32_t* chunk_len, int64_t n_chunks,
                        const wgbsseg_params* P, const BorderAlloc& alloc, int64_t* borders_off, char* err, size_t errlen, bool allow_plain = true, EarlyOut* early = nullptr)
{
    if (!P || !borders_off) { set_err(err, errlen, "NULL params/borders pointer"); return WGBSSEG_E_ARG; }
    if (P->max_bp == 0) { set_err(err, errlen, "max_bp must be >= 1 (the reference reads uninitialised loci when it is 0: segmentor.cpp:38,114)"); return WGBSSEG_E_ARG; }
    if (P->max_cpg < 1) { set_err(err, errlen, "max_cpg must be >= 1"); return WGBSSEG_E_ARG; }
    int32_t longest = 1;
    if (chunk_len) for (int64_t i = 0; i < n_chunks; i++) longest = std::max(longest, chunk_len[i]);
    Batch b;
    b.c = c; b.chunk_start0 = chunk_start0; b.chunk_len = chunk_len; b.n_chunks = n_chunks;
    b.alloc = &alloc; b.borders_off = borders_off; b.early = early; b.allow_plain = allow_plain;
    b.P = *P;
    b.P.max_cpg = std::min<uint32_t>(P->max_cpg, (uint32_t)longest);
    if ((uint64_t)b.P.max_cpg * 255u >= (1u << 24) || b.P.max_cpg > WGBSSEG_MAX_CPG) {
        set_err(err, errlen, "max_cpg %u with chunks of up to %d sites unsupported: blocks of more than %d sites (255 * sites >= 2^24) do not keep their counts exact "
                "in the float sums of the reference itself (segmentor.cpp:122-123), and windows are stored in 16 bits", P->max_cpg, (int)longest, WGBSSEG_MAX_CPG);
        return WGBSSEG_E_ARG;
    }
    b.marks = c && c->batch_marks;
    b.mark(0);
    if (!(P->pseudo_count >= 0.0f)) { set_err(err, errlen, "pseudo_count must be >= 0"); return WGBSSEG_E_ARG; }
    if (c && c->batch_open) {
        HIP_TRY(hipSetDevice(c->device));
        HIP_TRY(hipDeviceSynchronize());
        c->out_pending = false;
    }
    if (c) c->batch_open = true;
    int rc = build_job(c, chunk_start0, chunk_len, n_chunks, b.job, true, err, errlen);
    if (rc != WGBSSEG_OK) return rc;
    rc = plan_validation(c, b.job, !c->accumulate, err, errlen);
    if (rc != WGBSSEG_OK) return rc;
    c->last_valid = false;
    b.nC = (int)n_chunks;
    b.J = b.job.sites;

    rc = b.front(err, errlen);
    if (rc != WGBSSEG_OK) return rc;
    if (b.st.loci_disorder || b.st.overflow) return b.disorder_exit(err, errlen);
    rc = plan_tiles(c, b.job, b.st, b.P.pseudo_count, b.plan, err, errlen);
    if (rc != WGBSSEG_OK) return rc;
    plan_stages(c, b.job, b.st, b.plan);
// ... 80 lines not shown
    HIP_TRY(hipStreamSynchronize(c->sA));
    HIP_TRY(hipMemcpyAsync(&st2, c->status.p, sizeof(st2), hipMemcpyDeviceToHost, c->sA));
    HIP_TRY(hipStreamSynchronize(c->sA));
    if (st2.first_bad != ~0ULL) return report_bad_site(c, st2, err, errlen);
    if (!st.loci_disorder) { set_err(err, errlen, "a chunk scores more than 2^32 blocks; use a smaller chunk_size"); return WGBSSEG_E_ARG; }
    if (!allow_plain) {
        set_err(err, errlen, "internal: loci not ascending inside chunk %u (0-based sites [%lld, +%d)) of a batch that was filtered for such chunks",
                st.loci_disorder - 1, (long long)(job.h[st.loci_disorder - 1].start0 + c->site_base), (int)job.h[st.loci_disorder - 1].len);
        return WGBSSEG_E_LOCI_ORDER;
    }
    DevBuf flags;
    HIP_TRY(flags.ensure((size_t)n_chunks * 4));
    HIP_TRY(hipMemsetAsync(flags.p, 0, (size_t)n_chunks * 4, c->sA));
    hipLaunchKernelGGL(k_find_disorder, dim3((unsigned)n_chunks), dim3(WG_BLOCK), 0, c->sA, job.v, flags.as<uint32_t>());
    HIP_TRY(hipGetLastError());
    std::vector<uint32_t> hf((size_t)n_chunks);
    HIP_TRY(hipMemcpyAsync(hf.data(), flags.p, (size_t)n_chunks * 4, hipMemcpyDeviceToHost, c->sA));
    HIP_TRY(hipStreamSynchronize(c->sA));
    std::vector<int64_t> os, ooff;
    std::vector<int32_t> ol, ob;
    for (int64_t i = 0; i < n_chunks; i++) if (!hf[(size_t)i]) { os.push_back(chunk_start0[i]); ol.push_back(chunk_len[i]); }
    if (!os.empty()) {
        ooff.resize(os.size() + 1);
        const int rc = segment_chunks_impl(c, os.data(), ol.data(), (int64_t)os.size(), &P,
                                           [&](int64_t total) { ob.resize((size_t)std::max<int64_t>(1, total)); return ob.data(); }, ooff.data(), err, errlen, false);
        if (rc != WGBSSEG_OK) return rc;
    }
    std::vector<std::vector<int32_t>> plain((size_t)n_chunks);
    for (int64_t i = 0; i < n_chunks; i++)
        if (hf[(size_t)i]) {
            wgbsseg_params Pc = P;
            const int rc = plain_segment_chunk(c, chunk_start0[i], chunk_len[i], &Pc, plain[(size_t)i], err, errlen);
            if (rc != WGBSSEG_OK) return rc;
        }
    int64_t total = 0;
    size_t oi = 0;
    for (int64_t i = 0; i < n_chunks; i++) {
        borders_off[i] = total;
        if (hf[(size_t)i]) total += (int64_t)plain[(size_t)i].size();
        else { total += ooff[oi + 1] - ooff[oi]; oi++; }
    }
    borders_off[n_chunks] = total;
    int32_t* out = (*alloc)(total);
    if (!out) { set_err(err, errlen, "borders_out too small: need %lld ints", (long long)total); return WGBSSEG_E_CAPACITY; }
    oi = 0;
    for (int64_t i = 0; i < n_chunks; i++) {
        if (hf[(size_t)i]) memcpy(out + borders_off[i], plain[(size_t)i].data(), plain[(size_t)i].size() * 4);
        else { memcpy(out + borders_off[i], ob.data() + ooff[oi], (size_t)(ooff[oi + 1] - ooff[oi]) * 4); oi++; }
    }
    c->last_valid = false;
    return WGBSSEG_OK;
}

int Batch::tile_plan(char* err, size_t errlen)
{
    BatchPlan& p = plan;
    const float pc = P.pseudo_count;
    const int n_stages = p.n_stages;
    CostArgs base;
    memset(&base, 0, sizeof(base));
    base.pc = pc; base.pc2 = pc + pc;
    base.xcd_group = 64;
    base.cmap = 3;
    for (int k = 0; k < 3; k++) { ca[k] = base; ca[k].NS = p.NS[k]; ca[k].rows = p.rows[k]; }
    if (p.term_mode[0] == 2) {
        const bool same = c->lookup_pc == pc && c->lookup_rows[0] == p.rows[0] && c->lookup_rows[1] == p.rows[1] && c->lookup_rows[2] == p.rows[2] && c->lookup.p;
        if (!same) {
            static const wg_log_tables host_tabs = WG_LOG_TABLES_INIT;
            c->h_lookup.resize((size_t)(p.rows[0] + p.rows[1] + p.rows[2]) * 80);
            wg_d2* dst = c->h_lookup.data();
            for (int rows : p.rows) {
                for (int x = 0; x < rows * 16; x++) dst[x] = wg_ks_iy_entry(&host_tabs, rows, x);
                for (int x = 0; x < rows * 64; x++) dst[rows * 16 + x] = wg_ks_ky_entry(&host_tabs, rows, x);
                dst += (size_t)rows * 80;
            }
            HIP_TRY(c->lookup.ensure(c->h_lookup.size() * sizeof(wg_d2)));
            HIP_TRY(hipMemcpyAsync(c->lookup.p, c->h_lookup.data(), c->h_lookup.size() * sizeof(wg_d2), hipMemcpyHostToDevice, c->sA));
            c->lookup_pc = pc;
            for (int k = 0; k < 3; k++) c->lookup_rows[k] = p.rows[k];
        }
        const wg_d2* tab = c->lookup.as<wg_d2>();
        for (int k = 0; k < 3; k++) { ca[k].tab = tab; tab += (size_t)p.rows[k] * 80; }
    }
    const size_t sb_bytes = (size_t)(n_stages + 1) * 4;
    HIP_TRY(c->plan_sb.ensure(sb_bytes));
    const void* src = p.sb;
    if (c->h_sb.ensure(sb_bytes)) { memcpy(c->h_sb.p, src, sb_bytes); src = c->h_sb.p; }
    HIP_TRY(hipMemcpyAsync(c->plan_sb.p, src, sb_bytes, hipMemcpyHostToDevice, c->sA));
    HIP_TRY(c->plan_cbase.ensure((size_t)n_stages * nC * 8));
    HIP_TRY(c->plan_cum0.ensure((size_t)n_stages * nC * 4));
    HIP_TRY(c->plan_tbase.ensure((size_t)n_stages * (nC + 1) * 8 * 3));
    HIP_TRY(c->plan_cnt.ensure((size_t)n_stages * nC * 4 * 3));
    HIP_TRY(c->plan_pairs.ensure((size_t)n_stages * 8));
    HIP_TRY(c->plan_tiles.ensure((size_t)n_stages * 8 * 3));
    PlanArgs pa = {c->plan_sb.as<int32_t>(), p.TI, p.WA, WG_WIDE_TK, n_stages, p.WMED};
    uint32_t* cntA = c->plan_cnt.as<uint32_t>();
    uint32_t* cntB = cntA + (size_t)n_stages * nC;
    uint32_t* cntM = cntB + (size_t)n_stages * nC;
    int64_t* tbaseA = c->plan_tbase.as<int64_t>();
    int64_t* tbaseB = tbaseA + (size_t)n_stages * (nC + 1);
    int64_t* tbaseM = tbaseB + (size_t)n_stages * (nC + 1);
    if (!p.all_narrow) {
        hipLaunchKernelGGL(k_tile_count, dim3((unsigned)nC, (unsigned)n_stages), dim3(WG_BLOCK), 0, c->sA, job.v, pa, cntA, cntB, cntM);
        HIP_TRY(hipGetLastError());
    }
    hipLaunchKernelGGL(k_stage_plan, dim3((unsigned)n_stages), dim3(WG_PLAN_BLOCK), 0, c->sA, job.v, pa, (const uint32_t*)(p.all_narrow ? nullptr : cntA),
                       (const uint32_t*)(p.all_narrow ? nullptr : cntB), (const uint32_t*)(p.all_narrow ? nullptr : cntM),
                       c->plan_cbase.as<int64_t>(), c->plan_cum0.as<uint32_t>(), tbaseA, tbaseB, tbaseM, c->plan_pairs.as<int64_t>(), c->plan_tiles.as<int64_t>());
    HIP_TRY(hipGetLastError());
    if (!p.all_narrow) {
        const bool check_div_m = c->divs_enabled && p.term_mode[2] == 2 && p.WMED > 0 && c->divs_m_pc != pc;
        int rc;
        if (check_div_m && (rc = queue_div_check(c, pc, WG_MEDIUM_WMAX, hst + 3, err, errlen)) != WGBSSEG_OK) return rc;
        HIP_TRY(hipMemcpyAsync(p.stage_pairs.data(), c->plan_pairs.p, (size_t)n_stages * 8, hipMemcpyDeviceToHost, c->sA));
        HIP_TRY(hipMemcpyAsync(p.stage_tiles.data(), c->plan_tiles.p, (size_t)n_stages * 24, hipMemcpyDeviceToHost, c->sA));
        HIP_TRY(hipStreamSynchronize(c->sA));
        if (check_div_m) {
            c->divs_m_ok = *reinterpret_cast<const unsigned int*>(&hst[3]) == 0u;
            c->divs_m_pc = pc;
            if (profiling()) fprintf(stderr, "[wgbsseg] short division core for pseudo count %g on the operand pairs of a MEDIUM tile: %s\n", (double)pc, c->divs_m_ok ? "verified on every pair" : "NOT exact, the full core stays");
        }
    }
    for (int k = 0; k < 3; k++) {
        tile0[k].assign((size_t)n_stages + 1, 0);
        for (int stg = 0; stg < n_stages; stg++) tile0[k][(size_t)stg + 1] = tile0[k][(size_t)stg] + p.stage_tiles[3 * (size_t)stg + k];
        if (tile0[k][(size_t)n_stages] > 0x7fffffffLL) { set_err(err, errlen, "too many scoring tiles in one call"); return WGBSSEG_E_ARG; }
    }
    for (int k = 0; k < 3; k++) HIP_TRY(c->tiles[k].ensure((size_t)std::max<int64_t>(1, tile0[k][(size_t)n_stages]) * sizeof(TileDesc)));
    for (int stg = 0; stg < n_stages; stg++) {
        hipLaunchKernelGGL(k_tile_emit, dim3((unsigned)nC), dim3(WG_BLOCK), 0, c->sA, job.v, pa, stg, tbaseA, tbaseB, tbaseM,
                           c->tiles[0].as<TileDesc>() + tile0[0][(size_t)stg], c->tiles[1].as<TileDesc>() + tile0[1][(size_t)stg],
                           c->tiles[2].as<TileDesc>() + tile0[2][(size_t)stg]);
        HIP_TRY(hipGetLastError());
    }
    if (p.gated) {
        HIP_TRY(c->stage_ctr.ensure((size_t)n_stages * 4));
        HIP_TRY(hipMemsetAsync(c->stage_ctr.p, 0, (size_t)n_stages * 4, c->sA));
    }
    HIP_TRY(hipEventRecord(c->ev[EV_PLAN], c->sA));
    if (p.gated) HIP_TRY(hipStreamWaitEvent(c->sA2, c->ev[EV_PLAN], 0));
    mark(4);
    return WGBSSEG_OK;
}

int Batch::stages(char* err, size_t errlen)
{
    const BatchPlan& p = plan;
    const JobView& v = job.v;
    const int n_stages = p.n_stages;
    const int64_t max_stage_pairs = std::max<int64_t>(1, *std::max_element(p.stage_pairs.begin(), p.stage_pairs.end()));
    for (int k = 0; k < p.nbuf; k++) HIP_TRY(c->cost[k].ensure((size_t)max_stage_pairs * 8));
    HIP_TRY(c->dpstate.ensure((size_t)nC * (size_t)p.state_stride * 8));
    HIP_TRY(c->tmp_borders.ensure((size_t)(job.sites_padded + nC) * 4));
    HIP_TRY(c->nb.ensure((size_t)nC * 4));
    out_head = (size_t)round_up((int64_t)(nC + 1) * 8, 16);
    c->out_par ^= 1;
    outb = &c->out_borders[c->out_par];
    HIP_TRY(outb->ensure(out_head + (size_t)(J + nC) * 4));
    for (auto* evs : {&c->ev_cost0, &c->ev_cost1, &c->ev_dp0, &c->ev_dp1, &c->ev_fork, &c->ev_join}) grow_events(*evs, n_stages);
    StageView sv;
    sv.cbase = c->plan_cbase.as<int64_t>(); sv.cum0 = c->plan_cum0.as<uint32_t>();
    sv.tbaseA = c->plan_tbase.as<int64_t>(); sv.tbaseB = sv.tbaseA + (size_t)n_stages * (nC + 1);
    sv.sb = c->plan_sb.as<int32_t>();
    DpArgs da = {p.ringN, {c->dp_wlean ? 0 : 1, 0, 0}};
#ifdef WGBSSEG_DP_TIMING
    da.pad[1] = (int)env_int("WGBSSEG_DP_DEBUG", 0);
#endif
    c->last_dp_chunks = nC; c->last_dp_stride = p.state_stride;
    const size_t lds_dp = 2 * 4096 * 8 + 128 * 8 + 64 * 12 + 16 + 1024 * 6;
    double* const dps = c->dpstate.as<double>();
    if (st.wide_units) HIP_TRY(hipStreamWaitEvent(c->sA, c->ev[EV_SCAN_END], 0));
    if (st.wide_units && p.gated) HIP_TRY(hipStreamWaitEvent(c->sA2, c->ev[EV_SCAN_END], 0));
    const bool divsA = c->divs_enabled && c->divs_ok && c->divs_pc == P.pseudo_count;
    const bool divsM = c->divs_enabled && c->divs_m_ok && c->divs_m_pc == P.pseudo_count;
    const int fast[3] = {p.term_mode[0] == 2 && divsA ? 3 : p.term_mode[0], p.term_mode[1], p.term_mode[2] == 2 && divsM ? 3 : p.term_mode[2]};
    for (int stg = 0; stg < n_stages; stg++) {
        const int64_t* const nt = &p.stage_tiles[3 * (size_t)stg];
        hipStream_t const sP = p.gated && (stg & 1) ? c->sA2 : c->sA;
        sv.stage = stg;
        double* cbuf = c->cost[stg % p.nbuf].as<double>();
        const bool side = nt[0] > 0 && (nt[1] > 0 || nt[2] > 0);
        hipStream_t const sSide = side ? (p.gated && (stg & 1) ? c->sA : c->sA2) : sP;
        if (stg >= p.nbuf) HIP_TRY(hipStreamWaitEvent(sP, c->ev_dp1[stg - p.nbuf], 0));
        if (p.gated) {
            const int64_t before = stg > 0 ? nt[-3] + nt[-2] + nt[-1] : 0;
            if (before > 0) {
                const double est_s = 10.0 * (double)p.stage_pairs[(size_t)stg - 1] * c->n_samples / 5e11;
                const long long max_ticks = (long long)(1e8 * std::min(2.0, std::max(0.005, est_s)));
                hipLaunchKernelGGL(k_stage_gate, dim3(1), dim3(64), 0, sP, (const uint32_t*)(c->stage_ctr.as<uint32_t>() + (stg - 1)),
                                   (uint32_t)std::max<int64_t>(1, before - c->stage_gate), max_ticks);
                HIP_TRY(hipGetLastError());
            }
            for (CostArgs& a : ca) a.finished = c->stage_ctr.as<uint32_t>() + stg;
        }
        HIP_TRY(hipEventRecord(c->ev_cost0[stg], sP));
        if (side) { HIP_TRY(hipEventRecord(c->ev_fork[stg], sP)); HIP_TRY(hipStreamWaitEvent(sSide, c->ev_fork[stg], 0)); }
        for (int k : {0, 2, 1})
            if (nt[k] > 0)
                HIP_TRY(launch_cost_class(k, fast[k], p.TI, v, sv, ca[k], c->tiles[k].as<TileDesc>() + tile0[k][(size_t)stg], nt[k], cbuf, p.lds[k], k == 0 ? sP : sSide));
        if (side) { HIP_TRY(hipEventRecord(c->ev_join[stg], sSide)); HIP_TRY(hipStreamWaitEvent(sP, c->ev_join[stg], 0)); }
        HIP_TRY(hipEventRecord(c->ev_cost1[stg], sP));
        HIP_TRY(hipStreamWaitEvent(c->sB, c->ev_cost1[stg], 0));
        HIP_TRY(hipEventRecord(c->ev_dp0[stg], c->sB));
        const bool dp16 = p.dp_mode == 0 && n_stages > 1 && stg + 1 < n_stages;
        if (dp16)                                  hipLaunchKernelGGL((k_dp16<3>), dim3((unsigned)nC), dim3(64 * 4), (size_t)(2 * 16 * 64 * 8 + WG_DP_META_RING * 6), c->sB, v, sv, cbuf, dps, p.state_stride);
        else if (p.dp_mode == 0 && p.all_narrow)   hipLaunchKernelGGL((k_dp<7, 64, true>), dim3((unsigned)nC), dim3(64 * 8), lds_dp, c->sB, v, sv, cbuf, da, dps, p.state_stride);
        else if (p.dp_mode == 0)                   hipLaunchKernelGGL((k_dp<7, 64>), dim3((unsigned)nC), dim3(64 * 8), lds_dp, c->sB, v, sv, cbuf, da, dps, p.state_stride);
        else if (p.dp_mode == 1)                   hipLaunchKernelGGL((k_dp<7, 32>), dim3((unsigned)nC), dim3(64 * 8), lds_dp, c->sB, v, sv, cbuf, da, dps, p.state_stride);
        else                                       hipLaunchKernelGGL((k_dp<15, 32>), dim3((unsigned)nC), dim3(64 * 16), lds_dp, c->sB, v, sv, cbuf, da, dps, p.state_stride);
        HIP_TRY(hipGetLastError());
        HIP_TRY(hipEventRecord(c->ev_dp1[stg], c->sB));
    }
    return WGBSSEG_OK;
}

int Batch::deliver(char* err, size_t errlen)
{
    int64_t* const d_boff = outb->as<int64_t>();
    int32_t* const d_bord = reinterpret_cast<int32_t*>(reinterpret_cast<char*>(outb->p) + out_head);
    HIP_TRY(hipEventRecord(c->ev[EV_TRACE0], c->sB));
    hipLaunchKernelGGL(k_trace, dim3((unsigned)nC), dim3(WG_BLOCK), 0, c->sB, job.v, c->tmp_borders.as<int32_t>(), c->nb.as<int32_t>());
    HIP_TRY(hipGetLastError());
    hipLaunchKernelGGL(k_border_offsets, dim3(1), dim3(WG_BLOCK), 0, c->sB, c->nb.as<int32_t>(), nC, d_boff);
    HIP_TRY(hipGetLastError());
    hipLaunchKernelGGL(k_gather_borders, dim3((unsigned)nC), dim3(WG_BLOCK), 0, c->sB, job.v, c->tmp_borders.as<int32_t>(), c->nb.as<int32_t>(),
                       (const int64_t*)d_boff, d_bord);
    HIP_TRY(hipGetLastError());
    HIP_TRY(hipEventRecord(c->ev[EV_TRACE1], c->sB));
    const size_t small_bytes = out_head + (size_t)(J + nC) * 4;
    const bool small = small_bytes <= (512u << 10);
    const int64_t n_lead = (early && !small && early->n_lead > 0 && early->n_lead <= nC) ? early->n_lead : 0;
    size_t rest_cap = 0;
    if (n_lead) for (int64_t i = n_lead; i < nC; i++) rest_cap += (size_t)job.h[(size_t)i].len + 1;
    const size_t edge_bytes = (size_t)n_lead * 2 * WG_EDGE * 4, rest_bytes = rest_cap * 4;
    if (n_lead) {
        HIP_TRY(c->edges.ensure(edge_bytes + rest_bytes + 16));
        hipLaunchKernelGGL(k_gather_edges, dim3((unsigned)nC), dim3(WG_BLOCK), 0, c->sB, (const int64_t*)d_boff, (const int32_t*)d_bord, (int)n_lead, c->edges.as<int32_t>(),
                           c->edges.as<int32_t>() + edge_bytes / 4);
        HIP_TRY(hipGetLastError());
        HIP_TRY(hipEventRecord(c->ev[EV_TRACE1], c->sB));
    }
    if (!c->h_out.ensure((small ? small_bytes : out_head) + edge_bytes + rest_bytes)) { set_err(err, errlen, "out of page-locked host memory"); return WGBSSEG_E_NOMEM; }
    HIP_TRY(hipMemcpyAsync(c->h_out.p, outb->p, small ? small_bytes : (size_t)(nC + 1) * 8, hipMemcpyDeviceToHost, c->sB));
    if (n_lead) HIP_TRY(hipMemcpyAsync(reinterpret_cast<char*>(c->h_out.p) + out_head, c->edges.p, edge_bytes + rest_bytes, hipMemcpyDeviceToHost, c->sB));
    if (small || n_lead) HIP_TRY(hipEventRecord(c->ev[EV_HOME], c->sB));
    mark(5);
    if (J >= (1 << 20)) {
        HIP_TRY(hipEventSynchronize(c->ev_dp1[plan.n_stages - 1]));
        wgstitch::Pool::get().heat();
    }
    HIP_TRY(hipStreamSynchronize(c->sB));
    memcpy(borders_off, c->h_out.p, (size_t)(nC + 1) * 8);
    const int64_t total_b = borders_off[nC];
    int32_t* borders_out = (*alloc)(total_b);
    if (!borders_out) { set_err(err, errlen, "borders_out too small: need %lld ints", (long long)total_b); return WGBSSEG_E_CAPACITY; }
    if (small) memcpy(borders_out, reinterpret_cast<const char*>(c->h_out.p) + out_head, (size_t)total_b * 4);
    else if (n_lead && early->dest_device_visible && (reinterpret_cast<uintptr_t>(borders_out) & 15) == 0) {
        const int64_t lead_b = borders_off[n_lead];
        HIP_TRY(hipStreamWaitEvent(c->sC, c->ev[EV_TRACE1], 0));
        hipLaunchKernelGGL(k_copy_out, dim3(512), dim3(WG_BLOCK), 0, c->sC, (const int32_t*)d_bord, borders_out, lead_b);
        HIP_TRY(hipGetLastError());
        HIP_TRY(hipEventRecord(c->evD, c->sC));
        c->out_pending = true;
        memcpy(borders_out + lead_b, reinterpret_cast<const char*>(c->h_out.p) + out_head + edge_bytes, (size_t)(total_b - lead_b) * 4);
        early->edges = reinterpret_cast<const int32_t*>(reinterpret_cast<const char*>(c->h_out.p) + out_head);
        early->pending = true;
    } else {
        HIP_TRY(hipMemcpyAsync(borders_out, d_bord, (size_t)total_b * 4, hipMemcpyDeviceToHost, c->sB));
        HIP_TRY(hipEventRecord(c->ev[EV_HOME], c->sB));
        HIP_TRY(hipStreamSynchronize(c->sB));
    }
    mark(6);
    HIP_TRY(hipEventSynchronize(c->evS));
    if (hst[2].first_bad != ~0ULL) return report_bad_site(c, hst[2], err, errlen);
    return WGBSSEG_OK;
}

int Batch::timings(char* err, size_t errlen)
{
    const int n_stages = plan.n_stages;
    const int64_t total_pairs = (int64_t)st.total_pairs;
    if (marks) {
        auto at = [&](hipEvent_t e) { float x = 0; (void)hipEventElapsedTime(&x, c->ev[EV_BEGIN], e); return (double)x; };
        if (n_stages > 1) {
            fprintf(stderr, "[wgbsseg] %d stages%s, bounds", n_stages, plan.gated ? " (gated: alternating scoring streams)" : "");
            for (int q = 0; q <= n_stages; q++) fprintf(stderr, " %d", (int)plan.sb[q]);
            fprintf(stderr, "\n");
        }
        fprintf(stderr, "[wgbsseg] batch of %d chunks, %lld sites: windows done %.3f | stats copied %.3f | scan pass (its own stream) %.3f .. %.3f | plan + tiles done %.3f | "
                "scoring %.3f .. %.3f | recurrence %.3f .. %.3f | trace %.3f .. %.3f | borders on the host %.3f\n", nC, (long long)J,
                at(c->ev[EV_WINDOWS]), at(c->ev[EV_STATS]), at(c->ev[EV_VALIDATE0]), at(c->ev[EV_SCAN_END]), at(c->ev[EV_PLAN]), at(c->ev_cost0[0]), at(c->ev_cost1[n_stages - 1]),
                at(c->ev_dp0[0]), at(c->ev_dp1[n_stages - 1]), at(c->ev[EV_TRACE0]), at(c->ev[EV_TRACE1]), at(c->ev[EV_HOME]));
    }
    wgbsseg_timings& T = c->tim;
    if (!c->accumulate) memset(&T, 0, sizeof(T));
    float ms = 0;
    if (st.wide_units) HIP_TRY(hipEventElapsedTime(&ms, c->ev[EV_SCAN0], c->ev[EV_SCAN1])); else HIP_TRY(hipEventElapsedTime(&ms, c->ev[EV_VALIDATE0], c->ev[EV_VALIDATE1]));
    T.scan_ms += ms;
    const int64_t scan_bytes = 2 * (st.wide_units ? J : job.val_sites) * c->n_samples;
    if (scan_bytes > T.scan_main_bytes) { T.scan_main_bytes = scan_bytes; T.scan_main_ms = ms; }
    HIP_TRY(hipEventElapsedTime(&ms, c->ev[EV_BEGIN], c->ev[EV_WINDOWS])); T.window_ms += ms;
    float cost_end = 0;
    for (int stg = 0; stg < n_stages; stg++) {
        float t0 = 0, t1 = 0;
        HIP_TRY(hipEventElapsedTime(&t0, c->ev[EV_BEGIN], c->ev_cost0[stg])); HIP_TRY(hipEventElapsedTime(&t1, c->ev[EV_BEGIN], c->ev_cost1[stg]));
        if (t1 > std::max(t0, cost_end)) T.cost_ms += t1 - std::max(t0, cost_end);
        cost_end = std::max(cost_end, t1);
        HIP_TRY(hipEventElapsedTime(&ms, c->ev_dp0[stg], c->ev_dp1[stg])); T.dp_ms += ms;
    }
    HIP_TRY(hipEventElapsedTime(&ms, c->ev[EV_TRACE0], c->ev[EV_TRACE1])); T.trace_ms += ms;
    HIP_TRY(hipEventElapsedTime(&ms, c->ev[EV_BEGIN], c->ev[EV_HOME])); T.total_ms += ms;
    T.sites += J; T.pairs += total_pairs; T.evals += total_pairs * c->n_samples;
    T.scan_bytes += scan_bytes; T.max_window = std::max<int32_t>(T.max_window, plan.Wmax);
    T.n_stages = std::max<int32_t>(T.n_stages, n_stages); T.scan_launches += 1;
    if (plan.term_mode[0] == 2 && c->divs_enabled && c->divs_ok && c->divs_pc == P.pseudo_count) T.div_short = 1;
    c->last_sites = J; c->last_pairs = total_pairs; c->last_stages = n_stages; c->last_valid = true;
    c->batch_open = false;
    if (marks) {
        hm[7] = wall_s();
        fprintf(stderr, "[wgbsseg]   host clock of the batch, us after entry: tables up %.0f | windows queued %.0f | statistics here %.0f | scoring's tiles queued %.0f | everything queued %.0f | results here %.0f | return %.0f\n",
                (hm[1] - hm[0]) * 1e6, (hm[2] - hm[0]) * 1e6, (hm[3] - hm[0]) * 1e6, (hm[4] - hm[0]) * 1e6, (hm[5] - hm[0]) * 1e6, (hm[6] - hm[0]) * 1e6, (hm[7] - hm[0]) * 1e6);
    }
    return WGBSSEG_OK;
}

}

extern "C" {

int wgbsseg_segment_chunks(wgbsseg_ctx* c, const int64_t* chunk_start0, const int32_t* chunk_len, int64_t n_chunks,
                           const wgbsseg_params* P, int32_t* borders_out, int64_t borders_cap, int64_t* borders_off,
                           char* err, size_t errlen)
{
    if (!borders_out) { set_err(err, errlen, "NULL borders pointer"); return WGBSSEG_E_ARG; }
    BorderAlloc alloc = [&](int64_t total) -> int32_t* { return total <= borders_cap ? borders_out : nullptr; };
    return segment_chunks_impl(c, chunk_start0, chunk_len, n_chunks, P, alloc, borders_off, err, errlen);
}

int wgbsseg_segment_chunks_host(const uint8_t* betas, int64_t n_samples, int64_t sample_pitch_bytes, int64_t n_sites_total,
                                const uint32_t* loci, const int64_t* chunk_start0, const int32_t* chunk_len, int64_t n_chunks,
                                const wgbsseg_params* params, int device, int32_t* borders_out, int64_t borders_cap,
                                int64_t* borders_off, char* err, size_t errlen)
{
    if (!betas || n_samples < 1 || sample_pitch_bytes < 2 * n_sites_total) { set_err(err, errlen, "bad beta buffer"); return WGBSSEG_E_ARG; }
    wgbsseg_ctx* c = nullptr;
    int rc = wgbsseg_create(device, &c, err, errlen);
    if (rc != WGBSSEG_OK) return rc;
    std::vector<const uint8_t*> ptrs((size_t)n_samples);
    for (int64_t s = 0; s < n_samples; s++) ptrs[(size_t)s] = betas + s * sample_pitch_bytes;
    rc = wgbsseg_set_betas_host(c, ptrs.data(), n_samples, n_sites_total, err, errlen);
    if (rc == WGBSSEG_OK) rc = wgbsseg_set_loci_host(c, loci, n_sites_total, err, errlen);
    if (rc == WGBSSEG_OK) rc = wgbsseg_segment_chunks(c, chunk_start0, chunk_len, n_chunks, params, borders_out, borders_cap, borders_off, err, errlen);
    wgbsseg_destroy(c);
    return rc;
}

}

namespace {
int run_ctx_batch(wgbsseg_ctx* c, const std::vector<int64_t>& st0, const std::vector<int32_t>& ln, const wgbsseg_params* P, int64_t slot,
                  bool accumulate, const int32_t*& flat, std::vector<int64_t>& off, std::unique_ptr<int32_t[]>& owned, std::string& msg, EarlyOut* early = nullptr)
{
    off.resize(st0.size() + 1);
    int32_t* dst = nullptr;
    BorderAlloc alloc = [&](int64_t total) -> int32_t* {
        if (c->pinned.size() <= (size_t)slot) c->pinned.resize((size_t)slot + 1);
        PinnedBuf& pb = c->pinned[(size_t)slot];
        dst = pb.ensure((size_t)std::max<int64_t>(total, 1) * 4) ? reinterpret_cast<int32_t*>(pb.p) : nullptr;
        if (early) early->dest_device_visible = dst != nullptr;
        if (!dst) { owned.reset(new int32_t[(size_t)std::max<int64_t>(total, 1)]); dst = owned.get(); }
        return dst;
    };
    char ebuf[512] = {0};
    const bool acc_before = c->accumulate;
    c->accumulate = accumulate;
    const int rc = segment_chunks_impl(c, st0.data(), ln.data(), (int64_t)st0.size(), P, alloc, off.data(), ebuf, sizeof(ebuf), true, early);
    c->accumulate = acc_before;
    if (rc != WGBSSEG_OK) { msg = ebuf; return rc; }
    flat = dst;
    return WGBSSEG_OK;
}

int map_stitch_rc(int rc, const std::string& msg, char* err, size_t errlen)
{
    if (rc == 0) return WGBSSEG_OK;
    set_err(err, errlen, "%s", msg.c_str());
    return rc == wgstitch::E_CAPACITY ? WGBSSEG_E_CAPACITY : (rc < -1 ? rc : WGBSSEG_E_ARG);
}
}

extern "C" {

int wgbsseg_segment_regions(wgbsseg_ctx* c, const int64_t* region_start, const int64_t* region_end, int64_t n_regions,
                            int64_t chunk_size, const wgbsseg_params* P, int32_t* borders_out, int64_t borders_cap,
                            int64_t* borders_off, int64_t* stats, char* err, size_t errlen)
{
    if (!c || !P) { set_err(err, errlen, "bad arguments to segment_regions"); return WGBSSEG_E_ARG; }
// ... 1789 lines not shown
```

Measured before the change: 1.124 billion.

## Plan stages as chunk-by-site rectangles with optional chunk grouping

Stage bounds are replaced by rectangles over a chunk range and a site range, and the planning logic moves into a new header. An optional chunk-group mode, enabled through an environment variable and off by default, splits long chunks into groups so that different groups run as separate pipelined stages. Kernels now launch only over the rectangle's chunk range rather than all chunks. In the all-narrow multi-stage case the planner also copies per-stage pair counts back to the host with a stream synchronize, and the stage gate's tick budget now uses the device's reported wall-clock rate instead of a fixed constant.

```diff
diff --git a/include/wgbsseg.h b/include/wgbsseg.h
--- a/include/wgbsseg.h
+++ b/include/wgbsseg.h
@@ -8,7 +8,7 @@
 extern "C" {
 #endif
 
-#define WGBSSEG_VERSION 270
+#define WGBSSEG_VERSION 271
 #define WGBSSEG_MAX_CPG 65535
 
 #define WGBSSEG_OK              0
@@ -46,6 +46,7 @@
     int32_t div_short;
     double  scan_main_ms;
     int64_t scan_main_bytes;
+    int32_t n_groups;
 } wgbsseg_timings;
 
 int wgbsseg_version(void);
diff --git a/wgbs_tools_amd/_lib.py b/wgbs_tools_amd/_lib.py
--- a/wgbs_tools_amd/_lib.py
+++ b/wgbs_tools_amd/_lib.py
@@ -14,7 +14,7 @@
 
 OK, E_ARG, E_METH_GT_COV, E_NOMEM, E_HIP, E_LOCI_ORDER, E_CAPACITY, E_STATE, E_IO = 0, -1, -2, -3, -4, -5, -6, -7, -8
 
-ABI_VERSION = 270
+ABI_VERSION = 271
 EXPORTS = ['wgbsseg_version', 'wgbsseg_device_count', 'wgbsseg_create', 'wgbsseg_destroy',
            'wgbsseg_set_betas_host', 'wgbsseg_set_betas_device', 'wgbsseg_set_loci_host', 'wgbsseg_set_loci_device',
            'wgbsseg_segment_chunks', 'wgbsseg_segment_regions', 'wgbsseg_segment_chunks_host', 'wgbsseg_prefix_sums', 'wgbsseg_scan_only',
@@ -68,7 +68,7 @@
                 ('trace_ms', C.c_double), ('total_ms', C.c_double), ('sites', C.c_int64), ('pairs', C.c_int64),
                 ('evals', C.c_int64), ('scan_bytes', C.c_int64), ('max_window', C.c_int32), ('n_stages', C.c_int32),
                 ('scan_launches', C.c_int32), ('div_short', C.c_int32), ('scan_main_ms', C.c_double),
-                ('scan_main_bytes', C.c_int64)]
+                ('scan_main_bytes', C.c_int64), ('n_groups', C.c_int32)]
 
     def as_dict(self):
         return {k: getattr(self, k) for k, _ in self._fields_}
diff --git a/wgbs_tools_amd/build.py b/wgbs_tools_amd/build.py
--- a/wgbs_tools_amd/build.py
+++ b/wgbs_tools_amd/build.py
@@ -10,7 +10,7 @@
 HIPFLAGS = ['--offload-arch=' + ARCH, '-O3', '-std=c++17', '-ffp-contract=off', '-fPIC', '-shared', '-pthread']
 
 TARGETS = {
-    'libwgbsseg.so': (['wgbsseg.hip'], ['owners.h', 'env.h', 'seg_kernels.h', 'block_plan.h', 'block_kernels.h', 'plain_dp.h', 'wave_prims.h', 'exact_log2.h', 'stitch.h', 'add_loci.h', 'table_io.h', 'pat_kernels.h', 'homog_kernels.h', 'bimodal_kernels.h', 'stats_kernels.h', 'pair_plan.h', 'pair_kernels.h', 'bed_fmt.h', 'bed_plan.h', 'bed_kernels.h', 'share_plan.h', '../../include/wgbsseg.h']),
+    'libwgbsseg.so': (['wgbsseg.hip'], ['owners.h', 'env.h', 'seg_kernels.h', 'block_plan.h', 'block_kernels.h', 'plain_dp.h', 'wave_prims.h', 'exact_log2.h', 'stitch.h', 'add_loci.h', 'table_io.h', 'pat_kernels.h', 'homog_kernels.h', 'bimodal_kernels.h', 'stats_kernels.h', 'pair_plan.h', 'pair_kernels.h', 'bed_fmt.h', 'bed_plan.h', 'bed_kernels.h', 'share_plan.h', 'stage_plan.h', '../../include/wgbsseg.h']),
     'libwgbssynth.so': (['synth.hip'], []),
 }
 
diff --git a/wgbs_tools_amd/csrc/seg_kernels.h b/wgbs_tools_amd/csrc/seg_kernels.h
--- a/wgbs_tools_amd/csrc/seg_kernels.h
+++ b/wgbs_tools_amd/csrc/seg_kernels.h
@@ -3,6 +3,7 @@
 #include <stddef.h>
 #include <stdint.h>
 #include "exact_log2.h"
+#include "stage_plan.h"
 #include "wave_prims.h"
 
 #ifndef WG_CARRY_SHIFT
@@ -87,8 +88,16 @@
     const int64_t* tbaseA;
     const int64_t* tbaseB;
     int32_t stage;
-    const int32_t* sb;
+    const StageRect* rect;
 };
+
+__device__ __forceinline__ bool wg_stage_span(const StageRect* __restrict__ rect, int stg, int c, int len, int& s0, int& s1)
+{
+    const StageRect r = rect[stg];
+    s0 = r.s0;
+    s1 = r.s1 < len ? r.s1 : len;
+    return c >= r.c_lo && c < r.c_hi && r.s0 < len;
+}
 
 __device__ __forceinline__ uint4 wg_load16_guarded(const uint8_t* row, int64_t abs_site, int64_t n_total)
 {
@@ -457,7 +466,7 @@
     }
 }
 
-struct PlanArgs { const int32_t* sb; int32_t TI, WA, TK, n_stages, WM; };
+struct PlanArgs { const StageRect* rect; int32_t TI, WA, TK, n_stages, WM; };
 
 struct TileDesc { int32_t chunk, ka, nk, et_lo; };
 
@@ -486,10 +495,9 @@
     const int tid = threadIdx.x, lane = tid & 63, wv = tid >> 6;
     const int c = blockIdx.x, stg = blockIdx.y;
     const ChunkDesc cd = J.chunks[c];
-    const int s0 = P.sb[stg];
+    int s0, s1;
     uint32_t a = 0, b = 0, m = 0;
-    if (s0 < cd.len) {
-        const int s1 = (P.sb[stg + 1] < cd.len) ? P.sb[stg + 1] : cd.len;
+    if (wg_stage_span(P.rect, stg, c, cd.len, s0, s1)) {
         const int nU = (s1 - s0 + P.TI - 1) / P.TI;
         for (int u = tid; u < nU; u += WG_BLOCK) {
             uint32_t na, nb, nm;
@@ -525,9 +533,8 @@
         uint32_t c0 = 0;
         if (c < nC) {
             const ChunkDesc cd = J.chunks[c];
-            const int64_t s0 = P.sb[stg];
-            if (s0 < cd.len) {
-                const int64_t s1 = (P.sb[stg + 1] < cd.len) ? P.sb[stg + 1] : cd.len;
+            int s0, s1;
+            if (wg_stage_span(P.rect, stg, c, cd.len, s0, s1)) {
                 c0 = J.cum32[cd.site_off + s0];
                 const uint64_t cend = (s1 < cd.len) ? (uint64_t)J.cum32[cd.site_off + s1] : (uint64_t)J.chunk_pairs[c];
                 sz = cend - c0;
@@ -573,12 +580,11 @@
 {
     __shared__ uint32_t wa[WG_BLOCK / 64], wb[WG_BLOCK / 64], wm[WG_BLOCK / 64];
     const int tid = threadIdx.x, lane = tid & 63, wv = tid >> 6;
-    const int c = blockIdx.x;
+    const int c = P.rect[stg].c_lo + (int)blockIdx.x;
     const int nC = J.n_chunks;
     const ChunkDesc cd = J.chunks[c];
-    const int s0 = P.sb[stg];
-    if (s0 >= cd.len) return;
-    const int s1 = (P.sb[stg + 1] < cd.len) ? P.sb[stg + 1] : cd.len;
+    int s0, s1;
+    if (!wg_stage_span(P.rect, stg, c, cd.len, s0, s1)) return;
     const int nU = (s1 - s0 + P.TI - 1) / P.TI;
     int64_t runA = tbaseA[(int64_t)stg * (nC + 1) + c], runB = tbaseB[(int64_t)stg * (nC + 1) + c], runM = tbaseM[(int64_t)stg * (nC + 1) + c];
     for (int base = 0; base < nU; base += WG_BLOCK) {
@@ -1371,12 +1377,11 @@
     const int wvl = (int)(threadIdx.x >> 6);
     const bool worker = wvl != 0;
     const int lw = wvl - 1;
-    const int c = blockIdx.x;
+    const int c = SV.rect[SV.stage].c_lo + (int)blockIdx.x;
     const int nC = J.n_chunks;
     const ChunkDesc cd = J.chunks[c];
-    const int s0 = SV.sb[SV.stage];
-    if (s0 >= cd.len) return;
-    const int s1 = (SV.sb[SV.stage + 1] < cd.len) ? SV.sb[SV.stage + 1] : cd.len;
+    int s0, s1;
+    if (!wg_stage_span(SV.rect, SV.stage, c, cd.len, s0, s1)) return;
     const int rmask = A.ringN - 1;
     double* gs = state + (int64_t)c * state_stride;
     double* pendB = gs + WG_DP_STATE_HDR;
@@ -1613,12 +1618,11 @@
     const int lane = threadIdx.x & 63;
     const bool worker = threadIdx.x >= 64;
     const int lw = (int)(threadIdx.x >> 6) - 1;
-    const int c = blockIdx.x;
+    const int c = SV.rect[SV.stage].c_lo + (int)blockIdx.x;
     const int nC = J.n_chunks;
     const ChunkDesc cd = J.chunks[c];
-    const int s0 = SV.sb[SV.stage];
-    if (s0 >= cd.len) return;
-    const int s1 = (SV.sb[SV.stage + 1] < cd.len) ? SV.sb[SV.stage + 1] : cd.len;
+    int s0, s1;
+    if (!wg_stage_span(SV.rect, SV.stage, c, cd.len, s0, s1)) return;
     double* gs = state + (int64_t)c * state_stride;
     const double* cb = cost + SV.cbase[(int64_t)SV.stage * nC + c];
     const uint32_t cum0 = SV.cum0[(int64_t)SV.stage * nC + c];
diff --git a/wgbs_tools_amd/csrc/stage_plan.h b/wgbs_tools_amd/csrc/stage_plan.h
--- /dev/null
+++ b/wgbs_tools_amd/csrc/stage_plan.h
@@ -0,0 +1,130 @@
+#pragma once
+#include <algorithm>
+#include <cmath>
+#include <cstdint>
+#include <vector>
+
+struct StageRect { int32_t s0, s1, c_lo, c_hi; };
+
+namespace wgstage {
+
+constexpr int LONG_CHUNK = 8192;
+constexpr int FEW_CHUNKS = 160;
+
+struct Knobs {
+    long long cost_budget_bytes = 6144LL << 20;
+    int force_stages = 0, stage_gate = 768, last_stage_pct = -1, force_dp_mode = 0;
+    int chunk_group = 0;
+    bool stage_gate_shared = false;
+    bool alone = true;
+    double stage_gate_wide_evals = 100000.0, stage_min_evals_per_step = 21000.0;
+    int64_t n_samples = 1;
+};
+
+struct Job {
+    const int32_t* len = nullptr;
+    int n_chunks = 0;
+    int max_len = 0;
+    int64_t sites = 0, total_pairs = 0;
+    int Wmax = 0, narrow_wmax = 60;
+    int TI = 64;
+};
+
+struct Plan {
+    std::vector<StageRect> rects;
+    int n_groups = 1;
+    bool gated = false, all_narrow = false;
+    int last_pct = 100;
+    int nbuf = 1;
+    std::vector<int64_t> stage_pairs, stage_tiles;
+};
+
+inline int64_t round_up64(int64_t x, int64_t m) { return (x + m - 1) / m * m; }
+
+inline void rect_counts(const Job& j, const StageRect& r, int64_t& sites_in, int64_t& tiles)
+{
+    sites_in = tiles = 0;
+    for (int c = r.c_lo; c < r.c_hi; c++) {
+        const int64_t s1 = std::min<int64_t>(r.s1, j.len[c]);
+        if (s1 > r.s0) { tiles += (s1 - r.s0 + j.TI - 1) / j.TI; sites_in += s1 - r.s0; }
+    }
+}
+
+inline void cut_sites(const Knobs& k, Plan& p, int c_lo, int c_hi, int max_len, int64_t pairs, int n_stages, bool gated)
+{
+    const double evals_per_step = (double)pairs * (double)k.n_samples / std::max<double>(1.0, (double)max_len);
+    p.last_pct = !gated ? 100 : (k.last_stage_pct > 0 ? k.last_stage_pct : (evals_per_step <= 52500.0 ? 300 : 100));
+    const double parts = n_stages > 1 ? (double)(n_stages - 1) + p.last_pct / 100.0 : 1.0;
+    const int S = (int)std::max<int64_t>(64, round_up64((int64_t)std::ceil((double)max_len / parts), 64));
+    n_stages = std::min<int>(n_stages, (max_len + S - 1) / S);
+    for (int q = 0; q < n_stages; q++) {
+        const int32_t s0 = (int32_t)std::min<int64_t>((int64_t)q * S, max_len);
+        const int32_t s1 = q + 1 < n_stages ? (int32_t)std::min<int64_t>((int64_t)(q + 1) * S, max_len) : (int32_t)max_len;
+        p.rects.push_back({s0, s1, c_lo, c_hi});
+    }
+}
+
+inline void plan(const Knobs& k, const Job& j, Plan& p)
+{
+    p = Plan();
+    const int64_t total_pairs = j.total_pairs;
+    const long long bytes = total_pairs * 8;
+    int n_stages = (int)std::max<long long>(1, (bytes + k.cost_budget_bytes - 1) / k.cost_budget_bytes);
+    const bool budget_bound = n_stages > 1;
+    int n_long = 0;
+    for (int c = 0; c < j.n_chunks; c++) n_long += j.len[c] >= LONG_CHUNK;
+    const bool worth = (double)total_pairs * (double)k.n_samples >= (double)j.max_len * k.stage_min_evals_per_step;
+    if (j.max_len >= LONG_CHUNK) n_stages = std::max(n_stages, n_long <= FEW_CHUNKS && worth ? 8 : 1);
+    if (k.force_stages > 0) n_stages = k.force_stages;
+    n_stages = std::min<int>(n_stages, std::max(1, (j.max_len + 63) / 64));
+    p.all_narrow = j.Wmax <= j.narrow_wmax;
+    const int group = std::max(0, k.chunk_group);
+    const bool by_chunks = group > 0 && n_long > group && p.all_narrow && !budget_bound && k.force_dp_mode == 0 && j.max_len >= LONG_CHUNK;
+    auto is_gated = [&](int stages, double evals_per_step) {
+        return k.stage_gate > 0 && stages > 1 && (p.all_narrow || evals_per_step >= k.stage_gate_wide_evals || k.stage_gate_shared) && (k.stage_gate_shared || k.alone);
+    };
+    if (!by_chunks) {
+        const double evals_per_step = (double)total_pairs * (double)k.n_samples / std::max<double>(1.0, (double)j.max_len);
+        p.gated = is_gated(n_stages, evals_per_step);
+        cut_sites(k, p, 0, j.n_chunks, j.max_len, total_pairs, n_stages, p.gated);
+    } else {
+        std::vector<int> first;
+        int seen = 0, after_last_long = 0;
+        for (int c = 0; c < j.n_chunks; c++) {
+            if (j.len[c] < LONG_CHUNK) continue;
+            if (seen % group == 0) first.push_back(first.empty() ? 0 : c);
+            seen++;
+            after_last_long = c + 1;
+        }
+        first.push_back(after_last_long);
+        const int n_groups = (int)first.size() - 1;
+        p.n_groups = n_groups;
+        p.gated = is_gated(2, 0.0);
+        if (after_last_long < j.n_chunks) cut_sites(k, p, after_last_long, j.n_chunks, *std::max_element(j.len + after_last_long, j.len + j.n_chunks), 0, 1, false);
+        for (int g = 0; g + 1 < n_groups; g++)
+            cut_sites(k, p, first[(size_t)g], first[(size_t)g + 1], *std::max_element(j.len + first[(size_t)g], j.len + first[(size_t)g + 1]), 0, 1, false);
+        const int lo = first[(size_t)n_groups - 1], hi = after_last_long;
+        const int max_len_g = *std::max_element(j.len + lo, j.len + hi);
+        int64_t sites_g = 0;
+        for (int c = lo; c < hi; c++) sites_g += j.len[c];
+        const int64_t pairs_g = (int64_t)((double)total_pairs * (double)sites_g / (double)std::max<int64_t>(1, j.sites));
+        const bool worth_g = (double)pairs_g * (double)k.n_samples >= (double)max_len_g * k.stage_min_evals_per_step;
+        int n_last = k.force_stages > 0 ? k.force_stages : (worth_g ? 8 : 1);
+        n_last = std::min<int>(n_last, std::max(1, (max_len_g + 63) / 64));
+        cut_sites(k, p, lo, hi, max_len_g, pairs_g, n_last, p.gated);
+    }
+    n_stages = (int)p.rects.size();
+    p.stage_pairs.assign((size_t)n_stages, 0);
+    p.stage_tiles.assign((size_t)n_stages * 3, 0);
+    if (p.all_narrow) {
+        for (int stg = 0; stg < n_stages; stg++) {
+            int64_t nt = 0, sites_in = 0;
+            rect_counts(j, p.rects[(size_t)stg], sites_in, nt);
+            p.stage_tiles[3 * (size_t)stg] = nt;
+            p.stage_pairs[(size_t)stg] = n_stages == 1 ? total_pairs : std::min<int64_t>(total_pairs, sites_in * std::max(j.Wmax, 1));
+        }
+    }
+    p.nbuf = n_stages > 1 ? (p.gated && n_stages > 2 ? 3 : 2) : 1;
+}
+
+}
diff --git a/wgbs_tools_amd/csrc/wgbsseg.hip b/wgbs_tools_amd/csrc/wgbsseg.hip
--- a/wgbs_tools_amd/csrc/wgbsseg.hip
+++ b/wgbs_tools_amd/csrc/wgbsseg.hip
@@ -109,6 +109,8 @@
     bool last_valid = false;
     long long cost_budget_bytes = 0;
     int force_stages = 0;
+    int chunk_group = 0;
+    double wall_clock_hz = 1e8;
     bool counted_live = false;
     double stage_gate_wide_evals = 100000.0, stage_min_evals_per_step = 21000.0;
     bool stage_gate_shared = false;
@@ -126,7 +128,7 @@
     PinnedBuf bed_home[2], bed_tot;
     Event bed_ev[2][4];
     double bed_len_ms = 0.0, bed_emit_ms = 0.0;
-    std::vector<int32_t> h_stage_bounds;
+    std::vector<StageRect> h_stage_rects;
     float divs_pc = -1.0f;
     bool divs_ok = false;
     int64_t last_dp_chunks = 0, last_dp_stride = 0;
@@ -389,6 +391,11 @@
     const long long budget_mb = env_int("WGBSSEG_COST_BUDGET_MB", 0);
     c->cost_budget_bytes = (budget_mb > 0 ? budget_mb : 6144LL) << 20;
     c->force_stages = (int)env_int("WGBSSEG_FORCE_STAGES", 0);
+    c->chunk_group = (int)env_int("WGBSSEG_CHUNK_GROUP", 0, 0, 1 << 20);
+    {
+        int khz = 0;
+        if (hipDeviceGetAttribute(&khz, hipDeviceAttributeWallClockRate, device) == hipSuccess && khz > 0) c->wall_clock_hz = 1e3 * khz;
+    }
     c->stage_gate = (int)env_int("WGBSSEG_STAGE_GATE", c->stage_gate, 0);
     c->stage_gate_shared = env_flag("WGBSSEG_STAGE_GATE_SHARED", false);
     c->stage_gate_wide_evals = env_double("WGBSSEG_STAGE_GATE_WIDE_EVALS", c->stage_gate_wide_evals);
@@ -795,7 +802,8 @@
     int n_stages = 1;
     bool gated = false;
     int last_pct = 100;
-    const int32_t* sb = nullptr;
+    int n_groups = 1;
+    const StageRect* rect = nullptr;
     bool all_narrow = false;
     std::vector<int64_t> stage_pairs, stage_tiles;
     int dp_mode = 0;
@@ -871,43 +879,25 @@
 
 void plan_stages(wgbsseg_ctx* c, const Job& job, const JobStatus& st, BatchPlan& p)
 {
-    const int64_t total_pairs = (int64_t)st.total_pairs;
-    const long long bytes = total_pairs * 8;
-    int n_stages = (int)std::max<long long>(1, (bytes + c->cost_budget_bytes - 1) / c->cost_budget_bytes);
-    int n_long = 0;
-    for (const ChunkDesc& d : job.h) n_long += d.len >= 8192;
-    const bool worth = (double)total_pairs * c->n_samples >= (double)job.max_len * c->stage_min_evals_per_step;
-    if (job.max_len >= 8192) n_stages = std::max(n_stages, n_long <= 160 && worth ? 8 : 1);
-    if (c->force_stages > 0) n_stages = c->force_stages;
-    n_stages = std::min<int>(n_stages, std::max(1, (job.max_len + 63) / 64));
-    p.all_narrow = p.Wmax <= WG_NARROW_WMAX;
-    const double evals_per_step = (double)total_pairs * c->n_samples / std::max<double>(1.0, (double)job.max_len);
-    p.gated = c->stage_gate > 0 && n_stages > 1 && (p.all_narrow || evals_per_step >= c->stage_gate_wide_evals || c->stage_gate_shared) &&
-              (c->stage_gate_shared || g_live_ctx[c->device & 63].load(std::memory_order_relaxed) == 1);
-    p.last_pct = !p.gated ? 100 : (c->last_stage_pct > 0 ? c->last_stage_pct : (evals_per_step <= 52500.0 ? 300 : 100));
-    const double parts = n_stages > 1 ? (double)(n_stages - 1) + p.last_pct / 100.0 : 1.0;
-    const int S = (int)round_up((int64_t)std::ceil((double)job.max_len / parts), 64);
-    n_stages = std::min<int>(n_stages, (job.max_len + S - 1) / S);
-    std::vector<int32_t>& sb = c->h_stage_bounds;
-    sb.resize((size_t)n_stages + 1);
-    for (int q = 0; q < n_stages; q++) sb[(size_t)q] = (int32_t)std::min<int64_t>((int64_t)q * S, job.max_len);
-    sb[(size_t)n_stages] = (int32_t)job.max_len;
-    p.sb = sb.data();
-    p.n_stages = n_stages;
-    p.stage_pairs.assign((size_t)n_stages, 0);
-    p.stage_tiles.assign((size_t)n_stages * 3, 0);
-    if (p.all_narrow) {
-        for (int stg = 0; stg < n_stages; stg++) {
-            int64_t nt = 0, sites_in = 0;
-            for (const ChunkDesc& d : job.h) {
-                const int64_t s0 = sb[(size_t)stg], s1 = std::min<int64_t>(sb[(size_t)stg + 1], d.len);
-                if (s1 > s0) { nt += (s1 - s0 + p.TI - 1) / p.TI; sites_in += s1 - s0; }
-            }
-            p.stage_tiles[3 * (size_t)stg] = nt;
-            p.stage_pairs[(size_t)stg] = n_stages == 1 ? total_pairs : std::min<int64_t>(total_pairs, sites_in * std::max(p.Wmax, 1));
-        }
-    }
-    p.nbuf = n_stages > 1 ? (p.gated && n_stages > 2 ? 3 : 2) : 1;
+    wgstage::Knobs k;
+    k.cost_budget_bytes = c->cost_budget_bytes; k.force_stages = c->force_stages; k.stage_gate = c->stage_gate; k.last_stage_pct = c->last_stage_pct;
+    k.force_dp_mode = c->force_dp_mode; k.chunk_group = c->chunk_group; k.stage_gate_shared = c->stage_gate_shared;
+    k.alone = g_live_ctx[c->device & 63].load(std::memory_order_relaxed) == 1;
+    k.stage_gate_wide_evals = c->stage_gate_wide_evals; k.stage_min_evals_per_step = c->stage_min_evals_per_step; k.n_samples = c->n_samples;
+    std::vector<int32_t> lens(job.h.size());
+    for (size_t i = 0; i < job.h.size(); i++) lens[i] = job.h[i].len;
+    wgstage::Job j;
+    j.len = lens.data(); j.n_chunks = (int)lens.size(); j.max_len = job.max_len; j.sites = job.sites; j.total_pairs = (int64_t)st.total_pairs;
+    j.Wmax = p.Wmax; j.narrow_wmax = WG_NARROW_WMAX; j.TI = p.TI;
+    wgstage::Plan sp;
+    wgstage::plan(k, j, sp);
+    c->h_stage_rects = sp.rects;
+    p.rect = c->h_stage_rects.data();
+    p.n_stages = (int)sp.rects.size();
+    p.n_groups = sp.n_groups;
+    p.gated = sp.gated; p.all_narrow = sp.all_narrow; p.last_pct = sp.last_pct; p.nbuf = sp.nbuf;
+    p.stage_pairs = std::move(sp.stage_pairs);
+    p.stage_tiles = std::move(sp.stage_tiles);
     p.dp_mode = std::max(p.Wmax > 512 ? 2 : (p.Wmax > 64 ? 1 : 0), c->force_dp_mode);
     p.ringN = p.dp_mode ? ceil_pow2(p.Wmax + 128) : 0;
     p.state_stride = round_up(WG_DP_STATE_HDR + (int64_t)p.ringN + (p.ringN + 1) / 2, 2);
@@ -1154,9 +1144,9 @@
         const wg_d2* tab = c->lookup.as<wg_d2>();
         for (int k = 0; k < 3; k++) { ca[k].tab = tab; tab += (size_t)p.rows[k] * 80; }
     }
-    const size_t sb_bytes = (size_t)(n_stages + 1) * 4;
+    const size_t sb_bytes = (size_t)n_stages * sizeof(StageRect);
     HIP_TRY(c->plan_sb.ensure(sb_bytes));
-    const void* src = p.sb;
+    const void* src = p.rect;
     if (c->h_sb.ensure(sb_bytes)) { memcpy(c->h_sb.p, src, sb_bytes); src = c->h_sb.p; }
     HIP_TRY(hipMemcpyAsync(c->plan_sb.p, src, sb_bytes, hipMemcpyHostToDevice, c->sA));
     HIP_TRY(c->plan_cbase.ensure((size_t)n_stages * nC * 8));
@@ -1165,7 +1155,7 @@
     HIP_TRY(c->plan_cnt.ensure((size_t)n_stages * nC * 4 * 3));
     HIP_TRY(c->plan_pairs.ensure((size_t)n_stages * 8));
     HIP_TRY(c->plan_tiles.ensure((size_t)n_stages * 8 * 3));
-    PlanArgs pa = {c->plan_sb.as<int32_t>(), p.TI, p.WA, WG_WIDE_TK, n_stages, p.WMED};
+    PlanArgs pa = {c->plan_sb.as<StageRect>(), p.TI, p.WA, WG_WIDE_TK, n_stages, p.WMED};
     uint32_t* cntA = c->plan_cnt.as<uint32_t>();
     uint32_t* cntB = cntA + (size_t)n_stages * nC;
     uint32_t* cntM = cntB + (size_t)n_stages * nC;
@@ -1200,7 +1190,8 @@
     }
     for (int k = 0; k < 3; k++) HIP_TRY(c->tiles[k].ensure((size_t)std::max<int64_t>(1, tile0[k][(size_t)n_stages]) * sizeof(TileDesc)));
     for (int stg = 0; stg < n_stages; stg++) {
-        hipLaunchKernelGGL(k_tile_emit, dim3((unsigned)nC), dim3(WG_BLOCK), 0, c->sA, job.v, pa, stg, tbaseA, tbaseB, tbaseM,
+        if (p.rect[stg].c_hi <= p.rect[stg].c_lo) continue;
+        hipLaunchKernelGGL(k_tile_emit, dim3((unsigned)(p.rect[stg].c_hi - p.rect[stg].c_lo)), dim3(WG_BLOCK), 0, c->sA, job.v, pa, stg, tbaseA, tbaseB, tbaseM,
                            c->tiles[0].as<TileDesc>() + tile0[0][(size_t)stg], c->tiles[1].as<TileDesc>() + tile0[1][(size_t)stg],
                            c->tiles[2].as<TileDesc>() + tile0[2][(size_t)stg]);
         HIP_TRY(hipGetLastError());
@@ -1208,6 +1199,10 @@
     if (p.gated) {
         HIP_TRY(c->stage_ctr.ensure((size_t)n_stages * 4));
         HIP_TRY(hipMemsetAsync(c->stage_ctr.p, 0, (size_t)n_stages * 4, c->sA));
+    }
+    if (p.all_narrow && n_stages > 1) {
+        HIP_TRY(hipMemcpyAsync(p.stage_pairs.data(), c->plan_pairs.p, (size_t)n_stages * 8, hipMemcpyDeviceToHost, c->sA));
+        HIP_TRY(hipStreamSynchronize(c->sA));
     }
     HIP_TRY(hipEventRecord(c->ev[EV_PLAN], c->sA));
     if (p.gated) HIP_TRY(hipStreamWaitEvent(c->sA2, c->ev[EV_PLAN], 0));
@@ -1233,7 +1228,7 @@
     StageView sv;
     sv.cbase = c->plan_cbase.as<int64_t>(); sv.cum0 = c->plan_cum0.as<uint32_t>();
     sv.tbaseA = c->plan_tbase.as<int64_t>(); sv.tbaseB = sv.tbaseA + (size_t)n_stages * (nC + 1);
-    sv.sb = c->plan_sb.as<int32_t>();
+    sv.rect = c->plan_sb.as<StageRect>();
     DpArgs da = {p.ringN, {c->dp_wlean ? 0 : 1, 0, 0}};
 #ifdef WGBSSEG_DP_TIMING
     da.pad[1] = (int)env_int("WGBSSEG_DP_DEBUG", 0);
@@ -1258,7 +1253,7 @@
             const int64_t before = stg > 0 ? nt[-3] + nt[-2] + nt[-1] : 0;
             if (before > 0) {
                 const double est_s = 10.0 * (double)p.stage_pairs[(size_t)stg - 1] * c->n_samples / 5e11;
-                const long long max_ticks = (long long)(1e8 * std::min(2.0, std::max(0.005, est_s)));
+                const long long max_ticks = (long long)(c->wall_clock_hz * std::min(2.0, std::max(0.005, est_s)));
                 hipLaunchKernelGGL(k_stage_gate, dim3(1), dim3(64), 0, sP, (const uint32_t*)(c->stage_ctr.as<uint32_t>() + (stg - 1)),
                                    (uint32_t)std::max<int64_t>(1, before - c->stage_gate), max_ticks);
                 HIP_TRY(hipGetLastError());
@@ -1275,11 +1270,13 @@
         HIP_TRY(hipStreamWaitEvent(c->sB, c->ev_cost1[stg], 0));
         HIP_TRY(hipEventRecord(c->ev_dp0[stg], c->sB));
         const bool dp16 = p.dp_mode == 0 && n_stages > 1 && stg + 1 < n_stages;
-        if (dp16)                                  hipLaunchKernelGGL((k_dp16<3>), dim3((unsigned)nC), dim3(64 * 4), (size_t)(2 * 16 * 64 * 8 + WG_DP_META_RING * 6), c->sB, v, sv, cbuf, dps, p.state_stride);
-        else if (p.dp_mode == 0 && p.all_narrow)   hipLaunchKernelGGL((k_dp<7, 64, true>), dim3((unsigned)nC), dim3(64 * 8), lds_dp, c->sB, v, sv, cbuf, da, dps, p.state_stride);
-        else if (p.dp_mode == 0)                   hipLaunchKernelGGL((k_dp<7, 64>), dim3((unsigned)nC), dim3(64 * 8), lds_dp, c->sB, v, sv, cbuf, da, dps, p.state_stride);
-        else if (p.dp_mode == 1)                   hipLaunchKernelGGL((k_dp<7, 32>), dim3((unsigned)nC), dim3(64 * 8), lds_dp, c->sB, v, sv, cbuf, da, dps, p.state_stride);
-        else                                       hipLaunchKernelGGL((k_dp<15, 32>), dim3((unsigned)nC), dim3(64 * 16), lds_dp, c->sB, v, sv, cbuf, da, dps, p.state_stride);
+        const unsigned nR = (unsigned)std::max(0, p.rect[stg].c_hi - p.rect[stg].c_lo);
+        if (nR == 0) {}
+        else if (dp16)                             hipLaunchKernelGGL((k_dp16<3>), dim3(nR), dim3(64 * 4), (size_t)(2 * 16 * 64 * 8 + WG_DP_META_RING * 6), c->sB, v, sv, cbuf, dps, p.state_stride);
+        else if (p.dp_mode == 0 && p.all_narrow)   hipLaunchKernelGGL((k_dp<7, 64, true>), dim3(nR), dim3(64 * 8), lds_dp, c->sB, v, sv, cbuf, da, dps, p.state_stride);
+        else if (p.dp_mode == 0)                   hipLaunchKernelGGL((k_dp<7, 64>), dim3(nR), dim3(64 * 8), lds_dp, c->sB, v, sv, cbuf, da, dps, p.state_stride);
+        else if (p.dp_mode == 1)                   hipLaunchKernelGGL((k_dp<7, 32>), dim3(nR), dim3(64 * 8), lds_dp, c->sB, v, sv, cbuf, da, dps, p.state_stride);
+        else                                       hipLaunchKernelGGL((k_dp<15, 32>), dim3(nR), dim3(64 * 16), lds_dp, c->sB, v, sv, cbuf, da, dps, p.state_stride);
         HIP_TRY(hipGetLastError());
         HIP_TRY(hipEventRecord(c->ev_dp1[stg], c->sB));
     }
@@ -1355,8 +1352,8 @@
     if (marks) {
         auto at = [&](hipEvent_t e) { float x = 0; (void)hipEventElapsedTime(&x, c->ev[EV_BEGIN], e); return (double)x; };
         if (n_stages > 1) {
-            fprintf(stderr, "[wgbsseg] %d stages%s, bounds", n_stages, plan.gated ? " (gated: alternating scoring streams)" : "");
-            for (int q = 0; q <= n_stages; q++) fprintf(stderr, " %d", (int)plan.sb[q]);
+            fprintf(stderr, "[wgbsseg] %d stages in %d chunk group%s%s, chunks x sites", n_stages, plan.n_groups, plan.n_groups == 1 ? "" : "s", plan.gated ? " (gated: alternating scoring streams)" : "");
+            for (int q = 0; q < n_stages; q++) fprintf(stderr, " [%d,%d)x[%d,%d)", (int)plan.rect[q].c_lo, (int)plan.rect[q].c_hi, (int)plan.rect[q].s0, (int)plan.rect[q].s1);
             fprintf(stderr, "\n");
         }
         fprintf(stderr, "[wgbsseg] batch of %d chunks, %lld sites: windows done %.3f | stats copied %.3f | scan pass (its own stream) %.3f .. %.3f | plan + tiles done %.3f | "
@@ -1384,7 +1381,7 @@
     HIP_TRY(hipEventElapsedTime(&ms, c->ev[EV_BEGIN], c->ev[EV_HOME])); T.total_ms += ms;
     T.sites += J; T.pairs += total_pairs; T.evals += total_pairs * c->n_samples;
     T.scan_bytes += scan_bytes; T.max_window = std::max<int32_t>(T.max_window, plan.Wmax);
-    T.n_stages = std::max<int32_t>(T.n_stages, n_stages); T.scan_launches += 1;
+    T.n_stages = std::max<int32_t>(T.n_stages, n_stages); T.n_groups = std::max<int32_t>(T.n_groups, plan.n_groups); T.scan_launches += 1;
     if (plan.term_mode[0] == 2 && c->divs_enabled && c->divs_ok && c->divs_pc == P.pseudo_count) T.div_short = 1;
     c->last_sites = J; c->last_pairs = total_pairs; c->last_stages = n_stages; c->last_valid = true;
     c->batch_open = false;
```

Result: no change. 1.120 billion (-0.4%).
